# agnusmaximus/DistributedMNIST

Hardware: AMD Instinct MI355X
Metric: images/sec (whole node), MNIST CNN sync-SGD (higher is better)
Workload: dtype bf16; 1 GPU; model=lenet, global_batch=1024, parallelism=dp1, mode=full_sync, mode_requested=full_sync, grad_dtype=fp32

## Files before the change

csrc/bindings.cpp:

```cpp

#include <torch/extension.h>
#include <ATen/hip/HIPContext.h>
#include <hip/hip_runtime.h>

#include "kernels.h"

namespace {

#define CHECK_BF16(t) TORCH_CHECK((t).scalar_type() == at::kBFloat16, #t " must be bf16")
#define CHECK_F32(t) TORCH_CHECK((t).scalar_type() == at::kFloat, #t " must be fp32")
#define CHECK_CONTIG(t) TORCH_CHECK((t).is_contiguous(), #t " must be contiguous")
#define CHECK_CUDA(t) TORCH_CHECK((t).is_cuda(), #t " must be on GPU")

const unsigned short* bf16_ptr(const torch::Tensor& t) {
  return reinterpret_cast<const unsigned short*>(t.data_ptr());
}
unsigned short* bf16_mut(torch::Tensor& t) {
  return reinterpret_cast<unsigned short*>(t.data_ptr());
}

hipStream_t cur_stream() {
  return at::hip::getCurrentHIPStream().stream();
}

int cdiv(int a, int b) { return (a + b - 1) / b; }

int pick_splitk(int mtiles, int ntiles, int ksteps) {
  int tiles = mtiles * ntiles;
  if (tiles >= 256 || ksteps <= 1) return 1;
  int want = std::min(ksteps, std::max(1, 512 / tiles));
  return want;
}

int clamp_splitk(int want, int ksteps) {
  int s = std::max(1, std::min(want, ksteps));
  int per = cdiv(ksteps, s);
  return cdiv(ksteps, per);
}

int dw_tr_level() {
  static int v = [] {
    const char* e = getenv("DMNIST_DW_TR");
    return e ? atoi(e) : 1;
  }();
  return v;
}
bool dw_tr_enabled() { return dw_tr_level() != 0; }

bool conv2_dw_slab_route(int H, int W, int Cin, int Cout) {
  return conv2_dw_slab_supported(H, W, Cin, Cout) && dw_tr_enabled() &&
         conv2_dw_slab_enabled() && !getenv("DMNIST_DW_SPREAD");
}

struct DwPlan { int tr, tbm, bn, splitk; };
DwPlan linear_dw_plan(int K, int N, int B) {
  const int ksteps = cdiv(B, 64);
  if (!(dw_tr_enabled() && K % 8 == 0 && N % 64 == 0)) {
    int bm = cdiv(K, 128) * cdiv(N, 128) >= 128 ? 128 : 64;
    int want = pick_splitk(cdiv(K, bm), cdiv(N, bm), cdiv(B, 32));
    return {0, bm, bm, clamp_splitk(want, ksteps)};
  }
  int bn = (N % 128 == 0) ? 128 : 64;
  DwPlan old{1, 128, bn,
             clamp_splitk(pick_splitk(cdiv(K, 128), cdiv(N, bn), cdiv(B, 32)),
                          ksteps)};
  if (const char* e = getenv("DMNIST_DW_PLAN")) {
    int tbm = 0, fbn = 0, sk = 0;
    if (sscanf(e, "%d,%d,%d", &tbm, &fbn, &sk) == 3 &&
        (tbm == 64 || tbm == 128) && (fbn == 64 || fbn == 128) &&
        N % fbn == 0)
      return {1, tbm, fbn, clamp_splitk(sk, ksteps)};
    return old;
  }
  if (cdiv(K, 64) * cdiv(N, 64) >= 256) {
    if (B < 1536) return {1, 64, 64, 1};
    if (B < 6144) return {1, 64, bn, clamp_splitk(2, ksteps)};
  }
  return old;
}

void launch_linear_dw(GemmParams& p, int K, int N, int B, hipStream_t s) {
  DwPlan pl = linear_dw_plan(K, N, B);
  p.splitk = pl.splitk;
  if (pl.tr) {
    bool sw = pl.splitk == 1 && ((uintptr_t)p.C & 15) == 0 && p.ldc % 4 == 0;
    gemm_dw_tr(p, pl.tbm, pl.bn, sw, s);
  } else {
    (pl.tbm == 128 ? gemm_dw_128 : gemm_dw_64)(p, s);
  }
}

torch::Tensor linear_act_fwd_impl(torch::Tensor x, torch::Tensor w,
                                  torch::Tensor b, bool relu, double p_keep,
                                  int64_t seed, int64_t offset,
                                  const long* offset_dev,
                                  const c10::optional<torch::Tensor>& wT) {
  CHECK_CUDA(x); CHECK_BF16(x); CHECK_CONTIG(x);
  CHECK_BF16(w); CHECK_CONTIG(w);
  CHECK_F32(b); CHECK_CONTIG(b);
  int M = x.size(0), K = x.size(1), N = w.size(1);
  TORCH_CHECK(w.size(0) == K, "w/x shape mismatch");
  auto y = torch::empty({M, N}, x.options());
  GemmParams p{};
  p.A = bf16_ptr(x);
  p.bias = b.data_ptr<float>();
  p.C = y.data_ptr(); p.amax = nullptr;
  p.M = M; p.N = N; p.K = K;
  p.lda = K; p.ldc = N;
  p.splitk = 1;
  p.p_keep = (float)p_keep; p.seed = (uint64_t)seed; p.offset = (uint64_t)offset;
  p.offset_dev = offset_dev;
  bool drop = p_keep < 1.0;
  TORCH_CHECK(!drop || relu, "dropout path requires relu epilogue");
  int g128 = cdiv(M, 128) * cdiv(N, 128);
  bool big = g128 >= 512;
  if (const char* e = getenv("DMNIST_FC_TILE")) big = atoi(e) >= 128;
  auto s = cur_stream();
  bool bt = wT.has_value() && wT->defined();
  int tiles64 = cdiv(M, 64) * cdiv(N, 64);
  int ksteps = cdiv(K, 64);
  if (!big && tiles64 < 256 && ksteps >= 16 &&
      !getenv("DMNIST_FC_NOSPLIT")) {
    int sk = std::min(ksteps, std::max(2, 512 / tiles64));
    auto acc = torch::empty({(int64_t)sk, (int64_t)M, (int64_t)N},
                            x.options().dtype(at::kFloat));
    p.C = acc.data_ptr();
    p.splitk = sk;
    const char* fe = getenv("DMNIST_FC_FIXUP");
    bool fixup = fe && atoi(fe) != 0 && N % 8 == 0;
    if (fixup) {
      static std::vector<torch::Tensor>* ws = new std::vector<torch::Tensor>(64);
      int dev = x.get_device();
      TORCH_CHECK(dev >= 0 && dev < 64, "linear_act_fwd: bad device index");
      if (!(*ws)[dev].defined()) {
        hipStreamCaptureStatus cap = hipStreamCaptureStatusNone;
        hipStreamIsCapturing(s, &cap);
        TORCH_CHECK(cap == hipStreamCaptureStatusNone,
                    "linear_act_fwd: first split-K call on a device allocates "
                    "its ticket workspace and must run outside graph capture");
        (*ws)[dev] = torch::zeros({256}, x.options().dtype(at::kInt));
      }
      p.tickets = reinterpret_cast<unsigned*>((*ws)[dev].data_ptr<int>());
      p.Y = bf16_mut(y);
      p.relu = relu ? 1 : 0;
    }
    if (bt) {
      CHECK_BF16((*wT)); CHECK_CONTIG((*wT));
      TORCH_CHECK(wT->size(0) == N && wT->size(1) == K, "wT shape mismatch");
      p.B = bf16_ptr(*wT); p.ldb = K;
      (fixup ? gemm_fwd_slices_fix_64_bt : gemm_fwd_slices_64_bt)(p, s);
    } else {
      p.B = bf16_ptr(w); p.ldb = N;
      (fixup ? gemm_fwd_slices_fix_64 : gemm_fwd_slices_64)(p, s);
    }
    if (!fixup)
      launch_fwd_epilogue(acc.data_ptr<float>(), b.data_ptr<float>(),
                          bf16_mut(y), M, N, sk, relu ? 1 : 0, (float)p_keep,
                          (uint64_t)seed, (uint64_t)offset, offset_dev, s);
    return y;
  }
  if (bt) {
    CHECK_BF16((*wT)); CHECK_CONTIG((*wT));
    TORCH_CHECK(wT->size(0) == N && wT->size(1) == K, "wT shape mismatch");
    p.B = bf16_ptr(*wT); p.ldb = K;
    if (drop) (big ? gemm_fwd_drop_128_bt : gemm_fwd_drop_64_bt)(p, s);
    else if (relu) (big ? gemm_fwd_relu_128_bt : gemm_fwd_relu_64_bt)(p, s);
    else (big ? gemm_fwd_bias_128_bt : gemm_fwd_bias_64_bt)(p, s);
  } else {
    p.B = bf16_ptr(w); p.ldb = N;
    if (drop) (big ? gemm_fwd_drop_128 : gemm_fwd_drop_64)(p, s);
    else if (relu) (big ? gemm_fwd_relu_128 : gemm_fwd_relu_64)(p, s);
    else (big ? gemm_fwd_bias_128 : gemm_fwd_bias_64)(p, s);
  }
  return y;
}

torch::Tensor linear_act_fwd(torch::Tensor x, torch::Tensor w, torch::Tensor b,
                             bool relu, double p_keep, int64_t seed,
                             int64_t offset,
                             c10::optional<torch::Tensor> wT) {
  return linear_act_fwd_impl(x, w, b, relu, p_keep, seed, offset, nullptr, wT);
}

torch::Tensor linear_act_fwd_dev(torch::Tensor x, torch::Tensor w,
                                 torch::Tensor b, bool relu, double p_keep,
                                 int64_t seed, torch::Tensor offset_dev,
                                 c10::optional<torch::Tensor> wT) {
  TORCH_CHECK(offset_dev.scalar_type() == at::kLong && offset_dev.is_cuda(),
              "offset_dev must be a cuda int64 tensor");
  return linear_act_fwd_impl(x, w, b, relu, p_keep, seed, 0,
                             offset_dev.data_ptr<long>(), wT);
}

std::vector<torch::Tensor> linear_act_bwd_impl(torch::Tensor dy, torch::Tensor x,
                                               torch::Tensor w, torch::Tensor y,
                                               bool relu, double p_keep,
                                               bool need_dx,
                                               torch::Tensor dw, torch::Tensor db) {
  CHECK_CUDA(dy); CHECK_BF16(dy); CHECK_CONTIG(dy);
  CHECK_BF16(x); CHECK_CONTIG(x);
  CHECK_BF16(w); CHECK_CONTIG(w);
  int B = x.size(0), K = x.size(1), N = w.size(1);
  auto s = cur_stream();
  if (!db.defined())
    db = torch::zeros({N}, x.options().dtype(at::kFloat));
  CHECK_F32(db); CHECK_CONTIG(db);
  torch::Tensor dyeff;
  bool mask = relu || p_keep < 1.0;
  if (mask) {
    dyeff = torch::empty_like(dy);
    launch_relu_drop_bwd(bf16_ptr(dy), bf16_ptr(y), bf16_mut(dyeff),
                         db.data_ptr<float>(), B, N,
                         (float)(1.0 / p_keep), 1, s);
  } else {
    dyeff = dy;
    launch_relu_drop_bwd(bf16_ptr(dy), bf16_ptr(y), bf16_mut(dyeff),
                         db.data_ptr<float>(), B, N, 1.0f, 0, s);
  }
  if (!dw.defined())
    dw = torch::zeros({K, N}, x.options().dtype(at::kFloat));
  CHECK_F32(dw); CHECK_CONTIG(dw);
  {
    GemmParams p{};
    p.A = bf16_ptr(x); p.B = bf16_ptr(dyeff);
    p.C = dw.data_ptr();
    p.M = K; p.N = N; p.K = B;
    p.lda = K;
    p.ldb = N; p.ldc = N;
    launch_linear_dw(p, K, N, B, s);
  }
  torch::Tensor dx;
  if (need_dx) {
    dx = torch::empty({B, K}, x.options());
    GemmParams p{};
    p.A = bf16_ptr(dyeff); p.B = bf16_ptr(w);
    p.C = dx.data_ptr();
    p.M = B; p.N = K; p.K = N;
    p.lda = N; p.ldb = N; p.ldc = K;
    p.splitk = 1;
    bool big = cdiv(B, 128) * cdiv(K, 128) >= 128;
    (big ? gemm_dx_128 : gemm_dx_64)(p, s);
  } else {
    dx = torch::empty({0}, x.options());
  }
  return {dx, dw, db};
}

std::vector<torch::Tensor> linear_act_bwd(torch::Tensor dy, torch::Tensor x,
                                          torch::Tensor w, torch::Tensor y,
                                          bool relu, double p_keep,
                                          bool need_dx) {
  return linear_act_bwd_impl(dy, x, w, y, relu, p_keep, need_dx,
                             torch::Tensor(), torch::Tensor());
}

torch::Tensor linear_act_bwd_into(torch::Tensor dy, torch::Tensor x,
                                  torch::Tensor w, torch::Tensor y,
                                  bool relu, double p_keep, bool need_dx,
                                  torch::Tensor dw_out, torch::Tensor db_out) {
  auto r = linear_act_bwd_impl(dy, x, w, y, relu, p_keep, need_dx,
                               dw_out.view({x.size(1), w.size(1)}), db_out);
  return r[0];
}

std::vector<torch::Tensor> conv_pool_fwd(torch::Tensor x, torch::Tensor w,
                                         torch::Tensor b,
                                         c10::optional<torch::Tensor> wT) {
  CHECK_CUDA(x); CHECK_BF16(x); CHECK_CONTIG(x);
  CHECK_BF16(w); CHECK_CONTIG(w);
  CHECK_F32(b); CHECK_CONTIG(b);
  int NB = x.size(0), H = x.size(1), W = x.size(2), Cin = x.size(3);
  TORCH_CHECK(w.dim() == 4 && w.size(0) == 5 && w.size(1) == 5 &&
              w.size(2) == Cin, "conv weight must be [5,5,Cin,Cout]");
  int Cout = w.size(3);
  int Ho = H / 2, Wo = W / 2;
  auto y = torch::empty({NB, Ho, Wo, Cout}, x.options());
  auto amax = torch::empty({NB, Ho, Wo, Cout}, x.options().dtype(at::kByte));
  GemmParams p{};
  p.A = bf16_ptr(x); p.B = bf16_ptr(w);
  p.bias = b.data_ptr<float>();
  p.C = y.data_ptr(); p.amax = amax.data_ptr<uint8_t>();
  p.M = NB * Ho * Wo * 4; p.N = Cout; p.K = 25 * Cin;
  p.ldb = Cout; p.ldc = Cout;
  p.splitk = 1;
  p.CB = NB; p.CH = H; p.CW = W; p.CHo = Ho; p.CWo = Wo;
  p.Cin = Cin; p.Cout = Cout;
  auto s = cur_stream();
  if (Cin == 1 && conv1_mfma_supported(H, W, Cin, Cout) &&
      conv1_mfma_enabled() &&
      reinterpret_cast<uintptr_t>(x.data_ptr()) % 8 == 0) {
    launch_conv1_mfma_fwd(bf16_ptr(x), bf16_ptr(w), b.data_ptr<float>(),
                          bf16_mut(y), amax.data_ptr<uint8_t>(), NB, s);
  } else if (Cin == 1) {
    launch_conv1_direct_fwd(bf16_ptr(x), bf16_ptr(w), b.data_ptr<float>(),
                            bf16_mut(y), amax.data_ptr<uint8_t>(), NB, H, W,
                            Cout, s);
  } else if (conv_slab_supported(H, W, Cin, Cout)) {
    launch_conv_fwd_slab(bf16_ptr(x), bf16_ptr(w), b.data_ptr<float>(),
                         bf16_mut(y), amax.data_ptr<uint8_t>(), NB, H, W,
                         Cin, Cout, s);
  } else {
    TORCH_CHECK(Cin % 8 == 0, "conv requires Cin==1 or Cin%8==0");
    if (wT.has_value() && wT->defined()) {
      CHECK_BF16((*wT)); CHECK_CONTIG((*wT));
      p.B = bf16_ptr(*wT); p.ldb = 25 * Cin;
      conv_fwd_pool_bt(p, s);
    } else {
      conv_fwd_pool(p, s);
    }
  }
  return {y, amax};
}

std::vector<torch::Tensor> conv_pool_bwd_impl(torch::Tensor dy, torch::Tensor x,
                                              torch::Tensor w, torch::Tensor y,
                                              torch::Tensor amax, bool need_dx,
                                              torch::Tensor dw, torch::Tensor db) {
  CHECK_CUDA(dy); CHECK_BF16(dy); CHECK_CONTIG(dy);
  CHECK_BF16(x); CHECK_CONTIG(x); CHECK_BF16(w); CHECK_CONTIG(w);
  int NB = x.size(0), H = x.size(1), W = x.size(2), Cin = x.size(3);
  int Cout = w.size(3);
  int Ho = H / 2, Wo = W / 2;
  auto s = cur_stream();
  auto dact = torch::empty({NB, H, W, Cout}, x.options());
  if (!db.defined())
    db = torch::zeros({Cout}, x.options().dtype(at::kFloat));
  CHECK_F32(db); CHECK_CONTIG(db);
  launch_pool_bwd_scatter(bf16_ptr(dy), bf16_ptr(y),
                          amax.data_ptr<uint8_t>(), bf16_mut(dact),
                          db.data_ptr<float>(), NB * Ho * Wo, Cout, H, W, Wo,
                          s);
  if (!dw.defined())
    dw = torch::zeros({5, 5, Cin, Cout}, x.options().dtype(at::kFloat));
  CHECK_F32(dw); CHECK_CONTIG(dw);
  {
    GemmParams p{};
    p.A = bf16_ptr(x); p.B = bf16_ptr(dact);
    p.C = dw.data_ptr();
    p.M = 25 * Cin; p.N = Cout; p.K = NB * H * W;
    p.ldb = Cout; p.ldc = Cout;
    p.CB = NB; p.CH = H; p.CW = W; p.Cin = Cin; p.Cout = Cout;
    if (Cin == 1 && H <= 28 && W <= 28 && Cout <= 32 &&
        !getenv("DMNIST_DW1_SLAB")) {
      launch_conv1_dw_direct(bf16_ptr(x), bf16_ptr(dact),
                             dw.data_ptr<float>(), NB, H, W, Cout, s);
    } else if (Cin == 1 && conv1_slab_supported(H, W, Cin, Cout)) {
      launch_conv1_dw_slab(bf16_ptr(x), bf16_ptr(dact), dw.data_ptr<float>(),
                           NB, H, W, Cout, s);
    } else if (Cin == 1) {
      p.splitk = std::min(cdiv(p.K, 64), 2048);
      conv1_dw_gemm(p, s);
    } else if (conv_slab_supported(H, W, Cin, Cout) &&
               ((dw_tr_level() == 0 && NB >= 2048) || getenv("DMNIST_DW_G"))) {
      launch_conv_dw_slab(bf16_ptr(x), bf16_ptr(dact), dw.data_ptr<float>(),
                          NB, H, W, Cin, Cout, s);
    } else if (conv2_dw_slab_route(H, W, Cin, Cout)) {
      launch_conv2_dw_slab(bf16_ptr(x), bf16_ptr(dact), dw.data_ptr<float>(),
                           NB, s);
    } else {
      int tiles = cdiv(p.M, 128) * cdiv(p.N, 64);
      int want = p.K <= 262144 ? 1024 : 2048;
      if (const char* e = getenv("DMNIST_DW_BLOCKS")) want = atoi(e);
      p.splitk = std::min(cdiv(p.K, 64), std::max(1, want / tiles));
      if (dw_tr_enabled() && Cin % 8 == 0 && Cout % 64 == 0)
        conv_dw_tr(p, s);
      else
        conv_dw_gemm(p, s);
    }
  }
  torch::Tensor dx;
  if (need_dx && conv_slab_supported(H, W, Cin, Cout)) {
    dx = torch::empty({NB, H, W, Cin}, x.options());
    launch_conv_dx_slab(bf16_ptr(dact), bf16_ptr(w), bf16_mut(dx), NB, H, W,
                        Cin, Cout, s);
  } else if (need_dx) {
    TORCH_CHECK(Cout % 32 == 0, "conv_dx requires Cout%32==0");
    dx = torch::empty({NB, H, W, Cin}, x.options());
    GemmParams p{};
    p.A = bf16_ptr(dact); p.B = bf16_ptr(w);
    p.C = dx.data_ptr();
    p.M = NB * H * W; p.N = Cin; p.K = 25 * Cout;
    p.ldc = Cin;
    p.CB = NB; p.CH = H; p.CW = W; p.Cin = Cin; p.Cout = Cout;
    p.splitk = 1;
    conv_dx_gemm(p, s);
  } else {
    dx = torch::empty({0}, x.options());
  }
  return {dx, dw, db};
}

std::vector<torch::Tensor> conv_pool_bwd(torch::Tensor dy, torch::Tensor x,
                                         torch::Tensor w, torch::Tensor y,
                                         torch::Tensor amax, bool need_dx) {
  return conv_pool_bwd_impl(dy, x, w, y, amax, need_dx, torch::Tensor(),
                            torch::Tensor());
}

torch::Tensor conv_pool_bwd_into(torch::Tensor dy, torch::Tensor x,
                                 torch::Tensor w, torch::Tensor y,
                                 torch::Tensor amax, bool need_dx,
                                 torch::Tensor dw_out, torch::Tensor db_out) {
  auto r = conv_pool_bwd_impl(dy, x, w, y, amax, need_dx,
                              dw_out.view_as(w), db_out);
  return r[0];
}

torch::Tensor mask_db(torch::Tensor dy, torch::Tensor y, bool relu,
                      double p_keep, torch::Tensor db_out) {
  CHECK_CUDA(dy); CHECK_BF16(dy); CHECK_CONTIG(dy);
  CHECK_F32(db_out); CHECK_CONTIG(db_out);
  int B = dy.size(0), N = dy.size(1);
  auto s = cur_stream();
  bool mask = relu || p_keep < 1.0;
  torch::Tensor dyeff = mask ? torch::empty_like(dy) : dy;
  launch_relu_drop_bwd(bf16_ptr(dy), mask ? bf16_ptr(y) : bf16_ptr(dy),
                       bf16_mut(dyeff), db_out.data_ptr<float>(), B, N,
                       (float)(1.0 / p_keep), mask ? 1 : 0, s);
  return dyeff;
}

void linear_dw_into(torch::Tensor x, torch::Tensor dyeff,
                    torch::Tensor dw_out) {
  CHECK_BF16(x); CHECK_CONTIG(x); CHECK_BF16(dyeff); CHECK_CONTIG(dyeff);
  CHECK_F32(dw_out);
  int B = x.size(0), K = x.size(1), N = dyeff.size(1);
  GemmParams p{};
  p.A = bf16_ptr(x); p.B = bf16_ptr(dyeff);
  p.C = dw_out.data_ptr();
  p.M = K; p.N = N; p.K = B;
  p.lda = K; p.ldb = N; p.ldc = N;
  launch_linear_dw(p, K, N, B, cur_stream());
}

torch::Tensor linear_dx(torch::Tensor dyeff, torch::Tensor w) {
  CHECK_BF16(dyeff); CHECK_CONTIG(dyeff); CHECK_BF16(w); CHECK_CONTIG(w);
  int B = dyeff.size(0), N = dyeff.size(1), K = w.size(0);
  auto dx = torch::empty({B, K}, dyeff.options());
  GemmParams p{};
  p.A = bf16_ptr(dyeff); p.B = bf16_ptr(w);
  p.C = dx.data_ptr();
  p.M = B; p.N = K; p.K = N;
  p.lda = N; p.ldb = N; p.ldc = K;
  p.splitk = 1;
  bool big = cdiv(B, 128) * cdiv(K, 128) >= 128;
  (big ? gemm_dx_128 : gemm_dx_64)(p, cur_stream());
  return dx;
}

torch::Tensor linear_dx_unpool(torch::Tensor dyeff, torch::Tensor w,
                               torch::Tensor amax, torch::Tensor db_out,
                               int64_t Ho, int64_t Wo, int64_t C) {
  CHECK_BF16(dyeff); CHECK_CONTIG(dyeff); CHECK_BF16(w); CHECK_CONTIG(w);
  int B = dyeff.size(0), N = dyeff.size(1), K = w.size(0);
  TORCH_CHECK(K == Ho * Wo * C, "linear_dx_unpool: K != Ho*Wo*C");
  auto dact = torch::empty({B, 2 * (int)Ho, 2 * (int)Wo, (int)C},
                           dyeff.options());
  GemmParams p{};
  p.A = bf16_ptr(dyeff); p.B = bf16_ptr(w);
  p.C = dact.data_ptr();
  p.M = B; p.N = K; p.K = N;
  p.lda = N; p.ldb = N; p.ldc = K;
  p.splitk = 1;
  p.CHo = Ho; p.CWo = Wo; p.Cout = C;
  p.amax = amax.data_ptr<uint8_t>();
  p.db = db_out.defined() ? db_out.data_ptr<float>() : nullptr;
  const char* le = getenv("DMNIST_UNPOOL_LINES");
  p.unpool_lines = !(le && atoi(le) == 0) && C % 64 == 0 &&
                   ((uintptr_t)p.amax & 15) == 0 && ((uintptr_t)p.C & 15) == 0;
  bool big = cdiv(B, 128) * cdiv(K, 128) >= (p.unpool_lines ? 400 : 512);
  if (const char* e = getenv("DMNIST_UNPOOL_TILE")) big = atoi(e) >= 128;
  (big ? gemm_dx_unpool_128 : gemm_dx_unpool_64)(p, cur_stream());
  return dact;
}

torch::Tensor linear_dx_mask(torch::Tensor dyeff, torch::Tensor w,
                             torch::Tensor actm, torch::Tensor db_out,
                             double p_keep) {
  CHECK_BF16(dyeff); CHECK_CONTIG(dyeff); CHECK_BF16(w); CHECK_CONTIG(w);
  CHECK_BF16(actm); CHECK_CONTIG(actm);
  int B = dyeff.size(0), N = dyeff.size(1), K = w.size(0);
  TORCH_CHECK(actm.size(0) == B && actm.size(1) == K, "actm shape mismatch");
  auto dx = torch::empty({B, K}, dyeff.options());
  GemmParams p{};
  p.A = bf16_ptr(dyeff); p.B = bf16_ptr(w);
  p.C = dx.data_ptr();
  p.M = B; p.N = K; p.K = N;
  p.lda = N; p.ldb = N; p.ldc = K;
  p.splitk = 1;
  p.p_keep = (float)(1.0 / p_keep);
  p.actm = bf16_ptr(actm);
  p.db = db_out.defined() ? db_out.data_ptr<float>() : nullptr;
  bool big = cdiv(B, 128) * cdiv(K, 128) >= 128;
  (big ? gemm_dx_mask_128 : gemm_dx_mask_64)(p, cur_stream());
  return dx;
}

torch::Tensor pool_scatter(torch::Tensor dy, torch::Tensor y,
                           torch::Tensor amax, torch::Tensor db_out,
                           int64_t H, int64_t W) {
  CHECK_BF16(dy); CHECK_CONTIG(dy);
  int NB = dy.size(0), Ho = dy.size(1), Wo = dy.size(2), C = dy.size(3);
  auto dact = torch::empty({NB, (int)H, (int)W, C}, dy.options());
  launch_pool_bwd_scatter(bf16_ptr(dy), bf16_ptr(y),
                          amax.data_ptr<uint8_t>(), bf16_mut(dact),
                          db_out.data_ptr<float>(), NB * Ho * Wo, C, H, W,
                          Wo, cur_stream());
  return dact;
}

void conv_dw_into(torch::Tensor x, torch::Tensor dact, torch::Tensor dw_out) {
  CHECK_BF16(x); CHECK_CONTIG(x); CHECK_BF16(dact); CHECK_CONTIG(dact);
  int NB = x.size(0), H = x.size(1), W = x.size(2), Cin = x.size(3);
  int Cout = dact.size(3);
  auto s = cur_stream();
  GemmParams p{};
  p.A = bf16_ptr(x); p.B = bf16_ptr(dact);
  p.C = dw_out.data_ptr();
  p.M = 25 * Cin; p.N = Cout; p.K = NB * H * W;
  p.ldb = Cout; p.ldc = Cout;
  p.CB = NB; p.CH = H; p.CW = W; p.Cin = Cin; p.Cout = Cout;
  if (Cin == 1 && H <= 28 && W <= 28 && Cout <= 32 &&
      !getenv("DMNIST_DW1_SLAB")) {
    launch_conv1_dw_direct(bf16_ptr(x), bf16_ptr(dact),
                           dw_out.data_ptr<float>(), NB, H, W, Cout, s);
  } else if (Cin == 1 && conv1_slab_supported(H, W, Cin, Cout)) {
    launch_conv1_dw_slab(bf16_ptr(x), bf16_ptr(dact),
                         dw_out.data_ptr<float>(), NB, H, W, Cout, s);
  } else if (Cin == 1) {
    p.splitk = std::min(cdiv(p.K, 64), 2048);
    conv1_dw_gemm(p, s);
  } else if (conv_slab_supported(H, W, Cin, Cout) &&
             ((dw_tr_level() == 0 && NB >= 2048) || getenv("DMNIST_DW_G"))) {
    launch_conv_dw_slab(bf16_ptr(x), bf16_ptr(dact), dw_out.data_ptr<float>(),
                        NB, H, W, Cin, Cout, s);
  } else if (conv2_dw_slab_route(H, W, Cin, Cout)) {
    launch_conv2_dw_slab(bf16_ptr(x), bf16_ptr(dact),
                         dw_out.data_ptr<float>(), NB, s);
  } else {
    int tiles = cdiv(p.M, 128) * cdiv(p.N, 64);
    int want = p.K <= 262144 ? 1024 : 2048;
    if (const char* e = getenv("DMNIST_DW_BLOCKS")) want = atoi(e);
    p.splitk = std::min(cdiv(p.K, 64), std::max(1, want / tiles));
    if (getenv("DMNIST_DW_SPREAD")) {
      static torch::Tensor scratch;
      int64_t need = 16LL * p.M * p.N;
      if (!scratch.defined() || scratch.numel() < need)
        scratch = torch::zeros({need}, dact.options().dtype(at::kFloat));
      p.C = scratch.data_ptr();
      p.offset = 1;
    }
    if (dw_tr_enabled() && Cin % 8 == 0 && Cout % 64 == 0)
      conv_dw_tr(p, s);
    else
      conv_dw_gemm(p, s);
  }
}

void conv1_dw_pooled(torch::Tensor x, torch::Tensor dyp, torch::Tensor am,
                     torch::Tensor dw_out, torch::Tensor db_out) {
  CHECK_BF16(x); CHECK_CONTIG(x);
  CHECK_BF16(dyp); CHECK_CONTIG(dyp);
  int NB = x.size(0), H = x.size(1), W = x.size(2);
  int Cout = dyp.size(3);
  TORCH_CHECK(x.size(3) == 1 && H == 28 && W == 28 && Cout == 32 &&
                  dyp.size(1) == H / 2 && dyp.size(2) == W / 2,
              "conv1_dw_pooled: LeNet conv1 shapes only");
  CHECK_CONTIG(am); CHECK_F32(dw_out); CHECK_CONTIG(dw_out);
  if (conv1_mfma_supported(H, W, 1, Cout) && conv1_mfma_enabled() &&
      reinterpret_cast<uintptr_t>(x.data_ptr()) % 8 == 0) {
    launch_conv1_mfma_dw(bf16_ptr(x), bf16_ptr(dyp), am.data_ptr<uint8_t>(),
                         dw_out.data_ptr<float>(),
                         db_out.defined() ? db_out.data_ptr<float>() : nullptr,
                         NB, cur_stream());
    return;
  }
  launch_conv1_dw_pooled(bf16_ptr(x), bf16_ptr(dyp),
                         am.data_ptr<uint8_t>(), dw_out.data_ptr<float>(),
                         db_out.defined() ? db_out.data_ptr<float>() : nullptr,
                         NB, H, W, Cout, cur_stream());
}

torch::Tensor conv_dx(torch::Tensor dact, torch::Tensor w, int64_t Cin) {
  CHECK_BF16(dact); CHECK_CONTIG(dact); CHECK_BF16(w); CHECK_CONTIG(w);
  int NB = dact.size(0), H = dact.size(1), W = dact.size(2),
      Cout = dact.size(3);
  auto s = cur_stream();
  auto dx = torch::empty({NB, H, W, (int)Cin}, dact.options());
  if (conv_slab_supported(H, W, Cin, Cout)) {
    launch_conv_dx_slab(bf16_ptr(dact), bf16_ptr(w), bf16_mut(dx), NB, H, W,
                        Cin, Cout, s);
  } else {
    TORCH_CHECK(Cout % 32 == 0, "conv_dx requires Cout%32==0");
    GemmParams p{};
    p.A = bf16_ptr(dact); p.B = bf16_ptr(w);
    p.C = dx.data_ptr();
    p.M = NB * H * W; p.N = Cin; p.K = 25 * Cout;
    p.ldc = Cin;
    p.CB = NB; p.CH = H; p.CW = W; p.Cin = Cin; p.Cout = Cout;
    p.splitk = 1;
    conv_dx_gemm(p, s);
  }
  return dx;
}

std::vector<torch::Tensor> softmax_xent_fwd(torch::Tensor logits,
                                            torch::Tensor labels,
                                            c10::optional<torch::Tensor> db_out,
                                            double inv_n) {
  CHECK_CUDA(logits); CHECK_BF16(logits); CHECK_CONTIG(logits);
  TORCH_CHECK(labels.scalar_type() == at::kLong, "labels must be int64");
  CHECK_CONTIG(labels);
  int B = logits.size(0), C = logits.size(1);
  TORCH_CHECK(C <= 16, "softmax_xent kernel supports C<=16");
  TORCH_CHECK(B <= 256 * SOFTMAX_MAX_BLOCKS, "softmax_xent: batch too large");
  auto dl = torch::empty_like(logits);
  auto out = torch::empty({2}, logits.options().dtype(at::kFloat));
  static std::vector<torch::Tensor>* ws = new std::vector<torch::Tensor>(64);
  int dev = logits.get_device();
  TORCH_CHECK(dev >= 0 && dev < 64, "softmax_xent: bad device index");
  if (!(*ws)[dev].defined()) {
    hipStreamCaptureStatus cap = hipStreamCaptureStatusNone;
    hipStreamIsCapturing(cur_stream(), &cap);
    TORCH_CHECK(cap == hipStreamCaptureStatusNone,
                "softmax_xent_fwd: first call on a device allocates its "
                "workspace and must run outside graph capture");
    (*ws)[dev] = torch::zeros({2 * SOFTMAX_MAX_BLOCKS + 1},
                              logits.options().dtype(at::kFloat));
  }
  float* part = (*ws)[dev].data_ptr<float>();
  unsigned* ticket = reinterpret_cast<unsigned*>(part + 2 * SOFTMAX_MAX_BLOCKS);
  float* dbp = nullptr;
  if (db_out.has_value() && db_out->defined())
    dbp = db_out->data_ptr<float>();
  launch_softmax_xent(bf16_ptr(logits), labels.data_ptr<long>(),
                      bf16_mut(dl), out.data_ptr<float>(), B, C, dbp,
                      (float)inv_n, part, ticket, cur_stream());
  auto loss = out.select(0, 0);
  auto correct = out.select(0, 1);
  return {loss, correct, dl};
}

void sgd_step(torch::Tensor master, torch::Tensor grad, torch::Tensor shadow,
              bool has_shadow, double lr, double scale, double dc_keep,
              int64_t seed, int64_t offset,
              c10::optional<torch::Tensor> momentum, double mu) {
  CHECK_CUDA(master); CHECK_F32(master); CHECK_CONTIG(master);
  CHECK_F32(grad); CHECK_CONTIG(grad);
  float* mom = nullptr;
  if (momentum.has_value() && momentum->defined()) {
    CHECK_F32((*momentum)); CHECK_CONTIG((*momentum));
    mom = momentum->data_ptr<float>();
  }
  launch_sgd_step(master.data_ptr<float>(), grad.data_ptr<float>(),
                  has_shadow ? bf16_mut(shadow) : nullptr,
                  has_shadow ? 1 : 0, master.numel(),
                  (float)(lr * scale), (float)dc_keep, (uint64_t)seed,
                  (uint64_t)offset, mom, (float)mu, cur_stream());
}

void sgd_step_dev(torch::Tensor master, torch::Tensor grad,
                  torch::Tensor shadow, bool has_shadow,
                  torch::Tensor lr_scale_dev, double dc_keep, int64_t seed,
                  torch::Tensor offset_dev,
                  c10::optional<torch::Tensor> momentum, double mu,
                  bool zero_grad) {
  CHECK_CUDA(master); CHECK_F32(master); CHECK_CONTIG(master);
  CHECK_F32(grad); CHECK_CONTIG(grad);
  CHECK_F32(lr_scale_dev);
  float* mom = nullptr;
  if (momentum.has_value() && momentum->defined()) {
    CHECK_F32((*momentum)); CHECK_CONTIG((*momentum));
    mom = momentum->data_ptr<float>();
  }
  launch_sgd_step_dev(master.data_ptr<float>(), grad.data_ptr<float>(),
                      has_shadow ? bf16_mut(shadow) : nullptr,
                      has_shadow ? 1 : 0, master.numel(),
                      lr_scale_dev.data_ptr<float>(), (float)dc_keep,
                      (uint64_t)seed, offset_dev.data_ptr<long>(),
                      mom, (float)mu, zero_grad ? 1 : 0, cur_stream());
}

void transpose_bf16_batch(std::vector<torch::Tensor> srcs,
                          std::vector<torch::Tensor> dsts) {
  TORCH_CHECK(srcs.size() == dsts.size() && srcs.size() <= 4,
              "up to 4 transpose pairs");
  TransposeDesc d[4];
  for (size_t i = 0; i < srcs.size(); ++i) {
    CHECK_BF16(srcs[i]); CHECK_CONTIG(srcs[i]);
    CHECK_BF16(dsts[i]); CHECK_CONTIG(dsts[i]);
    d[i] = {bf16_ptr(srcs[i]), bf16_mut(dsts[i]),
            (int)srcs[i].size(0), (int)srcs[i].size(1)};
  }
  launch_transpose_bf16_batch(d, (int)srcs.size(), cur_stream());
}

void transpose_bf16_batch_adv(std::vector<torch::Tensor> srcs,
                              std::vector<torch::Tensor> dsts,
                              torch::Tensor step_dev,
                              torch::Tensor lr_scale_dev, double lr0,
                              double decay, int64_t decay_steps,
                              double inv_contrib) {
  TORCH_CHECK(srcs.size() == dsts.size() && srcs.size() <= 4,
              "up to 4 transpose pairs");
  TransposeDesc d[4];
  for (size_t i = 0; i < srcs.size(); ++i) {
    CHECK_BF16(srcs[i]); CHECK_CONTIG(srcs[i]);
    CHECK_BF16(dsts[i]); CHECK_CONTIG(dsts[i]);
    d[i] = {bf16_ptr(srcs[i]), bf16_mut(dsts[i]),
            (int)srcs[i].size(0), (int)srcs[i].size(1)};
  }
  launch_transpose_bf16_batch_adv(
      d, (int)srcs.size(), step_dev.data_ptr<long>(),
      lr_scale_dev.data_ptr<float>(), (float)lr0, (float)decay,
      (int)decay_steps, (float)inv_contrib, cur_stream());
}

void transpose_bf16(torch::Tensor src, torch::Tensor dst) {
  CHECK_CUDA(src); CHECK_BF16(src); CHECK_CONTIG(src);
  CHECK_BF16(dst); CHECK_CONTIG(dst);
  TORCH_CHECK(src.dim() == 2 && dst.size(0) == src.size(1) &&
              dst.size(1) == src.size(0), "transpose shape mismatch");
  launch_transpose_bf16(bf16_ptr(src), bf16_mut(dst), src.size(0),
                        src.size(1), cur_stream());
}

void step_advance(torch::Tensor step_dev, torch::Tensor lr_scale_dev,
                  double lr0, double decay, int64_t decay_steps,
                  double inv_contrib) {
  launch_step_advance(step_dev.data_ptr<long>(),
                      lr_scale_dev.data_ptr<float>(), (float)lr0,
                      (float)decay, (int)decay_steps, (float)inv_contrib,
                      cur_stream());
}

void grad_mask(torch::Tensor g, double keep, int64_t seed, int64_t step,
               int64_t rank, int64_t base,
               c10::optional<torch::Tensor> step_dev) {
  CHECK_CUDA(g); CHECK_F32(g); CHECK_CONTIG(g);
  TORCH_CHECK(base % 4 == 0,
              "grad_mask: slice base must be 16B-aligned so slice-wise "
              "masks compose to the whole-buffer mask");
  const long* sd = nullptr;
  if (step_dev.has_value() && step_dev->defined())
    sd = step_dev->data_ptr<long>();
  launch_grad_mask(g.data_ptr<float>(), g.numel(), base, (float)keep,
                   (uint64_t)seed, (uint64_t)step, (uint64_t)rank, sd,
                   cur_stream());
}

void batch_gather(torch::Tensor img_u8, torch::Tensor lab_u8,
                  torch::Tensor lut, torch::Tensor x, torch::Tensor y,
                  int64_t seed, int64_t step,
                  c10::optional<torch::Tensor> step_dev) {
  CHECK_CUDA(img_u8); CHECK_CONTIG(img_u8);
  CHECK_CUDA(lab_u8); CHECK_CONTIG(lab_u8);
  CHECK_CUDA(lut); CHECK_BF16(lut); CHECK_CONTIG(lut);
  CHECK_CUDA(x); CHECK_BF16(x); CHECK_CONTIG(x);
  CHECK_CUDA(y); CHECK_CONTIG(y);
  TORCH_CHECK(img_u8.scalar_type() == at::kByte &&
              lab_u8.scalar_type() == at::kByte,
              "batch_gather: images/labels must be uint8");
  TORCH_CHECK(y.scalar_type() == at::kLong, "batch_gather: y must be int64");
  const int64_t N = lab_u8.numel(), B = y.numel();
  TORCH_CHECK(N >= 1 && N < (int64_t(1) << 31),
              "batch_gather: N out of range");
  TORCH_CHECK(B >= 1 && B <= N, "batch_gather: batch size ", B,
              " must be in [1, N=", N, "]");
  TORCH_CHECK(img_u8.numel() == N * 784, "batch_gather: images must be [N,784]");
  TORCH_CHECK(x.numel() == B * 784, "batch_gather: x must hold B*784 values");
  TORCH_CHECK(lut.numel() == 256, "batch_gather: lut must have 256 entries");
  TORCH_CHECK(reinterpret_cast<uintptr_t>(img_u8.data_ptr()) % 8 == 0 &&
              reinterpret_cast<uintptr_t>(x.data_ptr()) % 16 == 0,
              "batch_gather: images must be 8B- and x 16B-aligned");
  const long* sd = nullptr;
  if (step_dev.has_value() && step_dev->defined()) {
    TORCH_CHECK(step_dev->is_cuda() && step_dev->scalar_type() == at::kLong &&
                step_dev->numel() >= 1, "batch_gather: step_dev must be a "
                "device int64 tensor");
    sd = step_dev->data_ptr<long>();
  } else {
    TORCH_CHECK(step >= 0, "batch_gather: step must be >= 0");
  }
  launch_batch_gather(img_u8.data_ptr<uint8_t>(), lab_u8.data_ptr<uint8_t>(),
                      bf16_ptr(lut), bf16_mut(x), y.data_ptr<long>(),
                      (uint32_t)N, (uint32_t)B, (uint64_t)seed,
                      (uint64_t)step, sd, cur_stream());
}

void batch_gather_aug(torch::Tensor img_u8, torch::Tensor lab_u8,
                      torch::Tensor lut, torch::Tensor table, torch::Tensor x,
                      torch::Tensor y, int64_t seed, int64_t step,
                      c10::optional<torch::Tensor> step_dev) {
  CHECK_CUDA(img_u8); CHECK_CONTIG(img_u8);
  CHECK_CUDA(lab_u8); CHECK_CONTIG(lab_u8);
  CHECK_CUDA(lut); CHECK_BF16(lut); CHECK_CONTIG(lut);
  CHECK_CUDA(table); CHECK_CONTIG(table);
  CHECK_CUDA(x); CHECK_BF16(x); CHECK_CONTIG(x);
  CHECK_CUDA(y); CHECK_CONTIG(y);
  TORCH_CHECK(img_u8.scalar_type() == at::kByte &&
              lab_u8.scalar_type() == at::kByte,
              "batch_gather_aug: images/labels must be uint8");
  TORCH_CHECK(y.scalar_type() == at::kLong,
              "batch_gather_aug: y must be int64");
  TORCH_CHECK(table.scalar_type() == at::kInt && table.dim() == 2 &&
              table.size(1) == 6 && table.size(0) >= 1 &&
              table.size(0) < (int64_t(1) << 31),
              "batch_gather_aug: table must be int32 [T >= 1, 6]");
  const int64_t N = lab_u8.numel(), B = y.numel();
  TORCH_CHECK(N >= 1 && N < (int64_t(1) << 31),
              "batch_gather_aug: N out of range");
  TORCH_CHECK(B >= 1 && B <= N, "batch_gather_aug: batch size ", B,
              " must be in [1, N=", N, "]");
  TORCH_CHECK(img_u8.numel() == N * 784,
              "batch_gather_aug: images must be [N,784]");
  TORCH_CHECK(x.numel() == B * 784,
              "batch_gather_aug: x must hold B*784 values");
  TORCH_CHECK(lut.numel() == 256,
              "batch_gather_aug: lut must have 256 entries");
  TORCH_CHECK(reinterpret_cast<uintptr_t>(img_u8.data_ptr()) % 8 == 0 &&
              reinterpret_cast<uintptr_t>(x.data_ptr()) % 16 == 0,
              "batch_gather_aug: images must be 8B- and x 16B-aligned");
  const long* sd = nullptr;
  if (step_dev.has_value() && step_dev->defined()) {
    TORCH_CHECK(step_dev->is_cuda() && step_dev->scalar_type() == at::kLong &&
                step_dev->numel() >= 1, "batch_gather_aug: step_dev must be "
                "a device int64 tensor");
    sd = step_dev->data_ptr<long>();
  } else {
    TORCH_CHECK(step >= 0, "batch_gather_aug: step must be >= 0");
  }
  launch_batch_gather_aug(img_u8.data_ptr<uint8_t>(),
                          lab_u8.data_ptr<uint8_t>(), bf16_ptr(lut),
                          table.data_ptr<int>(), (uint32_t)table.size(0),
                          bf16_mut(x), y.data_ptr<long>(), (uint32_t)N,
                          (uint32_t)B, (uint64_t)seed, (uint64_t)step, sd,
                          cur_stream());
}

void range_gather(torch::Tensor img_u8, torch::Tensor lab_u8,
                  torch::Tensor lut, torch::Tensor x, torch::Tensor y,
                  int64_t start, c10::optional<torch::Tensor> start_dev) {
  CHECK_CUDA(img_u8); CHECK_CONTIG(img_u8);
  CHECK_CUDA(lab_u8); CHECK_CONTIG(lab_u8);
  CHECK_CUDA(lut); CHECK_BF16(lut); CHECK_CONTIG(lut);
  CHECK_CUDA(x); CHECK_BF16(x); CHECK_CONTIG(x);
  CHECK_CUDA(y); CHECK_CONTIG(y);
  TORCH_CHECK(img_u8.scalar_type() == at::kByte &&
              lab_u8.scalar_type() == at::kByte,
              "range_gather: images/labels must be uint8");
  TORCH_CHECK(y.scalar_type() == at::kLong, "range_gather: y must be int64");
  const int64_t N = lab_u8.numel(), B = y.numel();
  TORCH_CHECK(N >= 1 && N < (int64_t(1) << 31),
              "range_gather: N out of range");
  TORCH_CHECK(B >= 1 && B < (int64_t(1) << 31),
              "range_gather: chunk size out of range");
  TORCH_CHECK(img_u8.numel() == N * 784, "range_gather: images must be [N,784]");
  TORCH_CHECK(x.numel() == B * 784, "range_gather: x must hold B*784 values");
  TORCH_CHECK(lut.numel() == 256, "range_gather: lut must have 256 entries");
  TORCH_CHECK(reinterpret_cast<uintptr_t>(img_u8.data_ptr()) % 8 == 0 &&
              reinterpret_cast<uintptr_t>(x.data_ptr()) % 16 == 0,
              "range_gather: images must be 8B- and x 16B-aligned");
  const long* sd = nullptr;
  if (start_dev.has_value() && start_dev->defined()) {
    TORCH_CHECK(start_dev->is_cuda() && start_dev->scalar_type() == at::kLong &&
                start_dev->numel() >= 1, "range_gather: start_dev must be a "
                "device int64 tensor");
    sd = start_dev->data_ptr<long>();
  } else {
    TORCH_CHECK(start >= 0, "range_gather: start must be >= 0");
  }
  launch_range_gather(img_u8.data_ptr<uint8_t>(), lab_u8.data_ptr<uint8_t>(),
                      bf16_ptr(lut), bf16_mut(x), y.data_ptr<long>(),
                      (uint32_t)N, (uint32_t)B, (uint64_t)start, sd,
                      cur_stream());
}

void softmax_eval(torch::Tensor logits, torch::Tensor labels,
                  torch::Tensor loss_sum, torch::Tensor counts,
                  c10::optional<torch::Tensor> pred,
                  c10::optional<torch::Tensor> cursor_dev) {
  CHECK_CUDA(logits); CHECK_BF16(logits); CHECK_CONTIG(logits);
  CHECK_CUDA(labels); CHECK_CONTIG(labels);
  CHECK_CUDA(loss_sum); CHECK_F32(loss_sum); CHECK_CONTIG(loss_sum);
  CHECK_CUDA(counts); CHECK_CONTIG(counts);
  TORCH_CHECK(logits.dim() == 2, "softmax_eval: logits must be [B,C]");
  TORCH_CHECK(labels.scalar_type() == at::kLong,
              "softmax_eval: labels must be int64");
  TORCH_CHECK(counts.scalar_type() == at::kInt,
              "softmax_eval: counts must be int32");
  const int64_t B = logits.size(0), C = logits.size(1);
  TORCH_CHECK(C >= 1 && C <= 16, "softmax_eval kernel supports 1<=C<=16");
  TORCH_CHECK(B >= 1 && B <= 256 * SOFTMAX_MAX_BLOCKS,
              "softmax_eval: batch out of range");
  TORCH_CHECK(labels.numel() == B, "softmax_eval: labels must be [B]");
  TORCH_CHECK(loss_sum.numel() >= 1, "softmax_eval: loss_sum must be [1]");
  TORCH_CHECK(counts.numel() == 2 + C * C,
              "softmax_eval: counts must hold 2 + C*C = ", 2 + C * C,
              " values");
  uint8_t* pp = nullptr;
  if (pred.has_value() && pred->defined()) {
    TORCH_CHECK(pred->is_cuda() && pred->scalar_type() == at::kByte &&
                pred->is_contiguous() && pred->numel() == B,
                "softmax_eval: pred must be a contiguous device uint8 [B]");
    pp = pred->data_ptr<uint8_t>();
  }
  long* cp = nullptr;
  if (cursor_dev.has_value() && cursor_dev->defined()) {
    TORCH_CHECK(cursor_dev->is_cuda() &&
                cursor_dev->scalar_type() == at::kLong &&
                cursor_dev->numel() >= 1, "softmax_eval: cursor_dev must be "
                "a device int64 tensor");
    cp = cursor_dev->data_ptr<long>();
  }
  static std::vector<torch::Tensor>* ws = new std::vector<torch::Tensor>(64);
  int dev = logits.get_device();
  TORCH_CHECK(dev >= 0 && dev < 64, "softmax_eval: bad device index");
  if (!(*ws)[dev].defined()) {
    hipStreamCaptureStatus cap = hipStreamCaptureStatusNone;
    hipStreamIsCapturing(cur_stream(), &cap);
    TORCH_CHECK(cap == hipStreamCaptureStatusNone,
                "softmax_eval: first call on a device allocates its "
                "workspace and must run outside graph capture");
    (*ws)[dev] = torch::zeros({SOFTMAX_MAX_BLOCKS + 1},
                              logits.options().dtype(at::kFloat));
  }
  float* part = (*ws)[dev].data_ptr<float>();
  unsigned* ticket = reinterpret_cast<unsigned*>(part + SOFTMAX_MAX_BLOCKS);
  launch_softmax_eval(bf16_ptr(logits), labels.data_ptr<long>(),
                      loss_sum.data_ptr<float>(), counts.data_ptr<int>(), pp,
                      cp, (int)B, (int)C, part, ticket, cur_stream());
}

}

PYBIND11_MODULE(TORCH_EXTENSION_NAME, m) {
  m.def("linear_act_fwd", &linear_act_fwd, "fused linear+bias+relu+dropout",
        py::arg("x"), py::arg("w"), py::arg("b"), py::arg("relu"),
        py::arg("p_keep"), py::arg("seed"), py::arg("offset"),
        py::arg("wT") = c10::nullopt);
  m.def("transpose_bf16", &transpose_bf16, "bf16 2-D transpose (wT refresh)");
  m.def("transpose_bf16_batch_adv", &transpose_bf16_batch_adv,
        "batched transposes + fused device step/LR advance (graph tail)");
  m.def("transpose_bf16_batch", &transpose_bf16_batch,
        "up to 4 transposes in one launch");
  m.def("mask_db", &mask_db, "relu/dropout grad mask + bias-grad column sums");
  m.def("linear_dw_into", &linear_dw_into, "dW = x^T dyeff into bucket view");
  m.def("linear_dx", &linear_dx, "dx = dyeff @ W^T");
  m.def("linear_dx_mask", &linear_dx_mask,
        "dx GEMM with fused relu/dropout mask + bias-grad column sums",
        py::arg("dyeff"), py::arg("w"), py::arg("actm"), py::arg("db_out"),
        py::arg("p_keep"));
  m.def("linear_dx_unpool", &linear_dx_unpool,
        "dx GEMM fused with maxpool2x2 backward scatter + conv db",
        py::arg("dyeff"), py::arg("w"), py::arg("amax"),
        py::arg("db_out"), py::arg("Ho"), py::arg("Wo"), py::arg("C"));
  m.def("linear_dw_plan", [](int64_t K, int64_t N, int64_t B) {
    DwPlan pl = linear_dw_plan((int)K, (int)N, (int)B);
    return std::make_tuple(pl.tbm, pl.bn, pl.splitk);
  }, "(tbm, bn, splitk) the fc dW launcher picks for x[B,K], dyeff[B,N]");
  m.def("pool_scatter", &pool_scatter, "maxpool bwd scatter + conv db");
  m.def("conv_dw_into", &conv_dw_into, "conv dW into bucket view");
  m.def("conv1_dw_pooled", &conv1_dw_pooled,
        "conv1 dW+db from the pooled gradient (pool bwd fused, no dact1)",
        py::arg("x"), py::arg("dyp"), py::arg("am"),
        py::arg("dw_out"), py::arg("db_out"));
  m.def("conv1_dw_group", [](int64_t NB) {
          return (int64_t)conv1_mfma_dw_group((int)NB);
        }, "images per block the MFMA conv1 dW launcher picks for batch NB");
  m.def("conv2_dw_group", [](int64_t NB) {
          return (int64_t)conv2_dw_group((int)NB);
        }, "images per block the slab conv2 dW launcher picks for batch NB");
  m.def("conv_dx", &conv_dx, "conv dX");
  m.def("linear_act_bwd", &linear_act_bwd, "linear backward (dx, dw, db)");
  m.def("linear_act_bwd_into", &linear_act_bwd_into,
        "linear backward accumulating dw/db into bucket views");
  m.def("conv_pool_fwd", &conv_pool_fwd, "fused conv5x5+bias+relu+maxpool",
        py::arg("x"), py::arg("w"), py::arg("b"), py::arg("wT") = c10::nullopt);
  m.def("conv_pool_bwd", &conv_pool_bwd, "conv+pool backward (dx, dw, db)");
  m.def("conv_pool_bwd_into", &conv_pool_bwd_into,
        "conv backward accumulating dw/db into bucket views");
  m.def("softmax_xent_fwd", &softmax_xent_fwd, "fused softmax-CE (+grad, +optional fc2 db, +optional acc-mean scale)",
        py::arg("logits"), py::arg("labels"),
        py::arg("db_out") = c10::nullopt, py::arg("inv_n") = 1.0);
  m.def("sgd_step", &sgd_step, "fused flat SGD(+momentum) apply",
        py::arg("master"), py::arg("grad"), py::arg("shadow"),
        py::arg("has_shadow"), py::arg("lr"), py::arg("scale"),
        py::arg("dc_keep"), py::arg("seed"), py::arg("offset"),
        py::arg("momentum") = c10::nullopt, py::arg("mu") = 0.0);
  m.def("sgd_step_dev", &sgd_step_dev,
        "SGD apply with device-side lr/offset (hipGraph-capturable); "
        "zero_grad clears the bucket in the same pass",
        py::arg("master"), py::arg("grad"), py::arg("shadow"),
        py::arg("has_shadow"), py::arg("lr_scale_dev"), py::arg("dc_keep"),
        py::arg("seed"), py::arg("offset_dev"),
        py::arg("momentum") = c10::nullopt, py::arg("mu") = 0.0,
        py::arg("zero_grad") = false);
  m.def("step_advance", &step_advance,
        "device-side staircase LR + step increment (inside the graph)");
  m.def("grad_mask", &grad_mask,
        "per-rank pre-aggregation drop-connect mask (in-place, philox; "
        "reference distributed_train.py:194-203)",
        py::arg("g"), py::arg("keep"), py::arg("seed"), py::arg("step"),
        py::arg("rank"), py::arg("base") = 0,
        py::arg("step_dev") = c10::nullopt);
  m.def("batch_gather", &batch_gather,
        "gather one training batch from the device-resident uint8 set "
        "(Feistel epoch permutation keyed on seed + step; LUT-normalised "
        "to bf16) into x [B,28,28,1] bf16 / y [B] int64",
        py::arg("img_u8"), py::arg("lab_u8"), py::arg("lut"), py::arg("x"),
        py::arg("y"), py::arg("seed"), py::arg("step"),
        py::arg("step_dev") = c10::nullopt);
  m.def("batch_gather_aug", &batch_gather_aug,
        "batch_gather with on-device affine augmentation: image j is warped "
        "(integer bilinear, zero background) by row aug_indices(seed, step, "
        "j) of the int32 [T,6] Q16 inverse-affine table before the LUT",
        py::arg("img_u8"), py::arg("lab_u8"), py::arg("lut"),
        py::arg("table"), py::arg("x"), py::arg("y"), py::arg("seed"),
        py::arg("step"), py::arg("step_dev") = c10::nullopt);
  m.def("range_gather", &range_gather,
        "sequential chunk [start, start+B) of the device-resident uint8 set "
        "(LUT-normalised to bf16) into x [B,28,28,1] bf16 / y [B] int64; "
        "rows past N are zero-filled with label -1",
        py::arg("img_u8"), py::arg("lab_u8"), py::arg("lut"), py::arg("x"),
        py::arg("y"), py::arg("start"),
        py::arg("start_dev") = c10::nullopt);
  m.def("softmax_eval", &softmax_eval,
        "evaluation statistics accumulated across launches: loss_sum[1] "
        "fp32, counts[2 + C*C] int32 (live, correct, confusion), optional "
        "pred[B] uint8 and cursor_dev += B; rows with a label outside "
        "[0, C) contribute to nothing",
        py::arg("logits"), py::arg("labels"), py::arg("loss_sum"),
        py::arg("counts"), py::arg("pred") = c10::nullopt,
        py::arg("cursor_dev") = c10::nullopt);
  m.def("linear_act_fwd_dev", &linear_act_fwd_dev,
        "linear fwd with device-side dropout offset",
        py::arg("x"), py::arg("w"), py::arg("b"), py::arg("relu"),
        py::arg("p_keep"), py::arg("seed"), py::arg("offset_dev"),
        py::arg("wT") = c10::nullopt);
}
```

csrc/common.h:

```cpp
#pragma once

#include <hip/hip_runtime.h>
#include <hip/hip_bf16.h>
#include <stdint.h>

typedef __attribute__((ext_vector_type(8))) short short8;
typedef __attribute__((ext_vector_type(4))) float f32x4;
typedef unsigned short ushort_t;

#define DEV __device__ __forceinline__

DEV float bf2f(ushort_t u) {
  union { uint32_t i; float f; } v;
  v.i = uint32_t(u) << 16;
  return v.f;
}

DEV ushort_t f2bf(float f) {
  union { float f; uint32_t i; } v;
  v.f = f;
  uint32_t lsb = (v.i >> 16) & 1;
  uint32_t rounded = v.i + 0x7FFFu + lsb;
  if ((v.i & 0x7F800000u) == 0x7F800000u) rounded = v.i;
  return ushort_t(rounded >> 16);
}

struct Philox4 {
  uint32_t x, y, z, w;
};

DEV uint32_t mulhilo(uint32_t a, uint32_t b, uint32_t* hi) {
  uint64_t p = uint64_t(a) * uint64_t(b);
  *hi = uint32_t(p >> 32);
  return uint32_t(p);
}

DEV Philox4 philox4x32(uint64_t seed, uint64_t offset, uint64_t idx) {
  uint32_t k0 = uint32_t(seed), k1 = uint32_t(seed >> 32);
  uint32_t c0 = uint32_t(idx), c1 = uint32_t(idx >> 32);
  uint32_t c2 = uint32_t(offset), c3 = uint32_t(offset >> 32);
  const uint32_t M0 = 0xD2511F53u, M1 = 0xCD9E8D57u;
  const uint32_t W0 = 0x9E3779B9u, W1 = 0xBB67AE85u;
#pragma unroll
  for (int r = 0; r < 10; ++r) {
    uint32_t h0, h1;
    uint32_t l0 = mulhilo(M0, c0, &h0);
    uint32_t l1 = mulhilo(M1, c2, &h1);
    uint32_t n0 = h1 ^ c1 ^ k0;
    uint32_t n1 = l1;
    uint32_t n2 = h0 ^ c3 ^ k1;
    uint32_t n3 = l0;
    c0 = n0; c1 = n1; c2 = n2; c3 = n3;
    k0 += W0; k1 += W1;
  }
  return {c0, c1, c2, c3};
}

DEV float philox_uniform(uint64_t seed, uint64_t offset, uint64_t idx) {
  Philox4 p = philox4x32(seed, offset, idx);
  return float(p.x) * (1.0f / 4294967296.0f);
}

DEV int cdiv(int a, int b) { return (a + b - 1) / b; }

DEV void glds16(const ushort_t* src, ushort_t* dst) {
  __builtin_amdgcn_global_load_lds(src, dst, 16, 0, 0);
}

DEV uint2 tr16_issue(unsigned a) {
  uint2 d;
  asm volatile("ds_read_b64_tr_b16 %0, %1 offset:0"
               : "=&v"(d) : "v"(a) : "memory");
  return d;
}

DEV short8 pack_wait(uint2 lo, uint2 hi) {
  union { unsigned u[4]; short8 s; } r;
  r.u[0] = lo.x; r.u[1] = lo.y; r.u[2] = hi.x; r.u[3] = hi.y;
  asm volatile("s_waitcnt lgkmcnt(0)" : "+v"(r.s));
  return r.s;
}

typedef short bf16x2_t __attribute__((__vector_size__(2 * sizeof(short))));
DEV float dot2bf(unsigned a, unsigned b, float c) {
  union U { unsigned u; bf16x2_t v; };
  U ua, ub;
  ua.u = a; ub.u = b;
  return __builtin_amdgcn_fdot2_f32_bf16(ua.v, ub.v, c, false);
}
```

csrc/conv2_dw_slab.hip:

```cpp

#include "common.h"
#include "kernels.h"
#include <stdlib.h>
#include <stdexcept>

#define C2_MG 8
#define C2_XIMG (14 * 14 * 32)
#define C2_DIMG (14 * 14 * 64)

static __device__ __align__(16) unsigned short c2_zero_page[8];

DEV int c2_xswz(int s) { return ((s >> 3) & 1) << 1; }
DEV int c2_dswz(int k) { return (((k >> 1) & 1) | (((k >> 3) & 1) << 1)) << 1; }

extern __shared__ __align__(16) ushort_t c2_lds[];

template <int KHB, int NBUF>
__global__ __launch_bounds__(256, (KHB == 1 && NBUF == 1) ? 3 : 1)
void conv2_dw_slab_kernel(const ushort_t* __restrict__ x,
                          const ushort_t* __restrict__ dact,
                          float* __restrict__ dw, int NB, int G) {
  constexpr int NRX = 13 + KHB;
  constexpr int XPIX = C2_MG + NRX * 16 + C2_MG;
  constexpr int NJOB = NRX + 28;
  constexpr int NQ = (NJOB + 3) / 4;
  constexpr int NKB = 5 / KHB;
  constexpr int KS_UNROLL = KHB == 1 ? 7 : 1;
  constexpr int BUF = XPIX * 32 + 224 * 64;
  ushort_t* const X = c2_lds;
  ushort_t* const D = c2_lds + XPIX * 32;

  const int tid = threadIdx.x;
  const int lane = tid & 63, wave = tid >> 6;
  const int wr = wave >> 1, wc = wave & 1;

  const int pos = blockIdx.x >> 3;
  const int grp = (pos / NKB) * 8 + (blockIdx.x & 7);
  const int kh0 = (pos % NKB) * KHB;
  const int img0 = grp * G;
  if (img0 >= NB) return;

  if (tid < 64 * NBUF) {
    int t = tid & 63;
    int o = (t < 32) ? t * 8 : (C2_MG + NRX * 16) * 32 + (t - 32) * 8;
    *reinterpret_cast<short8*>(X + (tid >> 6) * BUF + o) =
        short8{0, 0, 0, 0, 0, 0, 0, 0};
  }

  int soff[NQ];
#pragma unroll
  for (int q = 0; q < NQ; ++q) {
    int j = wave + 4 * q;
    soff[q] = -1;
    if (j < NRX) {
      int ir = j + kh0 - 2, px = lane >> 2;
      int lc = (lane & 3) ^ c2_xswz(C2_MG + j * 16 + px);
      if (px < 14 && ir >= 0 && ir < 14) soff[q] = (ir * 14 + px) * 32 + lc * 8;
    } else if (j < NJOB) {
      int jj = j - NRX;
      int h = jj >> 1, px = (jj & 1) * 8 + (lane >> 3);
      int lc = (lane & 7) ^ c2_dswz(h * 16 + px);
      if (px < 14) soff[q] = (h * 14 + px) * 64 + lc * 8;
    }
  }
  const auto issue = [&](int buf, int img) {
    const ushort_t* xi = x + (size_t)img * C2_XIMG;
    const ushort_t* di = dact + (size_t)img * C2_DIMG;
#pragma unroll
    for (int q = 0; q < NQ; ++q) {
      int j = wave + 4 * q;
      if (j < NRX) {
        const ushort_t* src = soff[q] >= 0 ? xi + soff[q] : c2_zero_page;
        glds16(src, X + buf * BUF + (C2_MG + j * 16) * 32);
      } else if (j < NJOB) {
        const ushort_t* src = soff[q] >= 0 ? di + soff[q] : c2_zero_page;
        glds16(src, D + buf * BUF + (j - NRX) * 8 * 64);
      }
    }
  };

  const int r0 = (lane >> 4) * 8 + ((lane & 15) >> 2);
  const int cp = (lane & 3) >> 1, off8 = (lane & 1) * 8;
  unsigned aaddr[5][2], baddr[2][2];
#pragma unroll
  for (int kw = 0; kw < 5; ++kw)
#pragma unroll
    for (int t = 0; t < 2; ++t) {
      int s = C2_MG + r0 + 4 * t + kw - 2;
      aaddr[kw][t] = (unsigned)(uintptr_t)X +
                     (unsigned)(s * 64 + (((wr * 2 + cp) ^ c2_xswz(s)) << 4) +
                                off8);
    }
#pragma unroll
  for (int ni = 0; ni < 2; ++ni)
#pragma unroll
    for (int t = 0; t < 2; ++t) {
      int k = r0 + 4 * t;
      baddr[ni][t] = (unsigned)(uintptr_t)D +
                     (unsigned)(k * 128 +
                                (((wc * 4 + ni * 2 + cp) ^ c2_dswz(k)) << 4) +
                                off8);
    }

  f32x4 acc[KHB][5][2];
#pragma unroll
  for (int a = 0; a < KHB; ++a)
#pragma unroll
    for (int b = 0; b < 5; ++b)
#pragma unroll
      for (int c = 0; c < 2; ++c) acc[a][b][c] = f32x4{0.f, 0.f, 0.f, 0.f};

  const int n = min(G, NB - img0);
  if (NBUF == 2) issue(0, img0);
  for (int g = 0; g < n; ++g) {
    if (NBUF == 1) {
      __syncthreads();
      issue(0, img0 + g);
    }
    asm volatile("s_waitcnt vmcnt(0)" ::: "memory");
    __syncthreads();
    if (NBUF == 2 && g + 1 < n) issue((g + 1) & 1, img0 + g + 1);
    const unsigned boff = (unsigned)((g & (NBUF - 1)) * BUF * 2);
#pragma unroll KS_UNROLL
    for (int ks = 0; ks < 7; ++ks) {
      uint2 br[2][2];
#pragma unroll
      for (int ni = 0; ni < 2; ++ni)
#pragma unroll
        for (int t = 0; t < 2; ++t)
          br[ni][t] = tr16_issue(baddr[ni][t] + boff + ks * (32 * 128));
#pragma unroll
      for (int khl = 0; khl < KHB; ++khl) {
        uint2 ar[5][2];
#pragma unroll
        for (int kw = 0; kw < 5; ++kw)
#pragma unroll
          for (int t = 0; t < 2; ++t)
            ar[kw][t] = tr16_issue(aaddr[kw][t] + boff +
                                   (ks * 32 + khl * 16) * 64);
        short8 af[5], bf[2];
#pragma unroll
        for (int kw = 0; kw < 5; ++kw) af[kw] = pack_wait(ar[kw][0], ar[kw][1]);
#pragma unroll
        for (int ni = 0; ni < 2; ++ni) bf[ni] = pack_wait(br[ni][0], br[ni][1]);
#pragma unroll
        for (int kw = 0; kw < 5; ++kw)
#pragma unroll
          for (int ni = 0; ni < 2; ++ni)
            acc[khl][kw][ni] = __builtin_amdgcn_mfma_f32_16x16x32_bf16(
                af[kw], bf[ni], acc[khl][kw][ni], 0, 0, 0);
      }
    }
  }

  const int frow = (lane >> 4) * 4, fcol = lane & 15;
#pragma unroll
  for (int khl = 0; khl < KHB; ++khl)
#pragma unroll
    for (int kw = 0; kw < 5; ++kw)
#pragma unroll
      for (int ni = 0; ni < 2; ++ni)
#pragma unroll
        for (int r = 0; r < 4; ++r) {
          int m = ((kh0 + khl) * 5 + kw) * 32 + wr * 16 + frow + r;
          int n = wc * 32 + ni * 16 + fcol;
          atomicAdd(dw + m * 64 + n, acc[khl][kw][ni][r]);
        }
}


bool conv2_dw_slab_supported(int H, int W, int Cin, int Cout) {
  return H == 14 && W == 14 && Cin == 32 && Cout == 64;
}

bool conv2_dw_slab_enabled() {
  const char* e = getenv("DMNIST_DW2_SLAB");
  return !(e && atoi(e) == 0);
}

int conv2_dw_group(int NB) {
  int G = NB >= 4096 ? 32 : (NB >= 512 ? 12 : (NB >= 128 ? 4 : 1));
  if (const char* e = getenv("DMNIST_DW2_G")) G = atoi(e);
  return G < 1 ? 1 : G;
}

template <int KHB, int NBUF>
static void c2_launch(const unsigned short* x, const unsigned short* dact,
                      float* dw, int NB, int G, int blocks, hipStream_t s) {
  constexpr int BYTES = NBUF * ((C2_MG * 2 + (13 + KHB) * 16) * 32 + 224 * 64) * 2;
  if (BYTES > 65536) {
    static const hipError_t granted = hipFuncSetAttribute(
        reinterpret_cast<const void*>(&conv2_dw_slab_kernel<KHB, NBUF>),
        hipFuncAttributeMaxDynamicSharedMemorySize, BYTES);
    if (granted != hipSuccess)
      throw std::runtime_error("conv2_dw_slab: LDS size not granted");
  }
  hipLaunchKernelGGL((conv2_dw_slab_kernel<KHB, NBUF>), dim3(blocks),
                     dim3(256), BYTES, s, x, dact, dw, NB, G);
}

void launch_conv2_dw_slab(const unsigned short* x, const unsigned short* dact,
                          float* dw, int NB, hipStream_t s) {
  if (NB <= 0) return;
  int G = conv2_dw_group(NB);
  int groups = (NB + G - 1) / G;
  int g8 = (groups + 7) / 8 * 8;
  const char* e = getenv("DMNIST_DW2_KHB");
  const char* b = getenv("DMNIST_DW2_NBUF");
  bool all_taps = e && atoi(e) == 5;
  int nbuf = b ? atoi(b) : 1;
  if (all_taps && nbuf == 2)
    c2_launch<5, 2>(x, dact, dw, NB, G, g8, s);
  else if (all_taps)
    c2_launch<5, 1>(x, dact, dw, NB, G, g8, s);
  else if (nbuf == 2)
    c2_launch<1, 2>(x, dact, dw, NB, G, g8 * 5, s);
  else
    c2_launch<1, 1>(x, dact, dw, NB, G, g8 * 5, s);
}
```

csrc/conv_slab.hip:

```cpp

#include "common.h"
#include "kernels.h"
#include <stdlib.h>

#define NTHREADS 256
#define BK 64
#define LDK (BK + 8)

typedef ushort_t u16;

__device__ __align__(16) static unsigned short g_zero_page_slab[8];

DEV short8 lds_row_shifted(const u16* row, int s) {
  int s0 = s & ~7;
  short8 lo = *reinterpret_cast<const short8*>(row + s0);
  short8 hi = *reinterpret_cast<const short8*>(row + s0 + 8);
  switch (s & 7) {
    case 0: return lo;
    case 1: return __builtin_shufflevector(lo, hi, 1, 2, 3, 4, 5, 6, 7, 8);
    case 2: return __builtin_shufflevector(lo, hi, 2, 3, 4, 5, 6, 7, 8, 9);
    case 3: return __builtin_shufflevector(lo, hi, 3, 4, 5, 6, 7, 8, 9, 10);
    case 4: return __builtin_shufflevector(lo, hi, 4, 5, 6, 7, 8, 9, 10, 11);
    case 5: return __builtin_shufflevector(lo, hi, 5, 6, 7, 8, 9, 10, 11, 12);
    case 6: return __builtin_shufflevector(lo, hi, 6, 7, 8, 9, 10, 11, 12, 13);
    default: return __builtin_shufflevector(lo, hi, 7, 8, 9, 10, 11, 12, 13, 14);
  }
}

template <int H, int W, int CIN, int COUT>
__global__ __launch_bounds__(NTHREADS)
void conv_fwd_slab_kernel(const u16* __restrict__ x,
                          const u16* __restrict__ w,
                          const float* __restrict__ bias, u16* __restrict__ y,
                          uint8_t* __restrict__ amax, int NB) {
  constexpr int HP = H + 4, WP = W + 4;
  constexpr int HO = H / 2, WO = W / 2;
  constexpr int M = HO * WO * 4;
  constexpr int BM = 224;
  constexpr int BN = COUT;
  constexpr int WM = 112, WN = BN / 2;
  constexpr int MI = WM / 16, NI = WN / 16;
  constexpr int K = 25 * CIN;
  constexpr int PST = CIN + 8;
  __shared__ __align__(16) u16 slab[HP * WP * PST];
  __shared__ __align__(16) u16 Bs[2][BK][BN];

  const int tid = threadIdx.x;
  const int lane = tid & 63;
  const int wave = tid >> 6;
  const int wr = wave >> 1, wc = wave & 1;
  const int img = blockIdx.x;
  const u16* xi = x + (size_t)img * H * W * CIN;

  constexpr int BLPR = BN / 8;
  constexpr int BQ = BN / 32;
  int bnc[BQ];
#pragma unroll
  for (int q = 0; q < BQ; ++q) {
    int rt = (wave * BQ + q) * (512 / BN) + lane / BLPR;
    int xs = (rt ^ (rt >> 3)) & (BLPR - 1);
    bnc[q] = ((lane % BLPR) ^ xs) * 8;
  }
  const auto issueB = [&](int buf, int kt) {
#pragma unroll
    for (int q = 0; q < BQ; ++q) {
      int row0 = (wave * BQ + q) * (512 / BN);
      int k = kt + row0 + lane / BLPR;
      const u16* src =
          (k < K) ? w + (size_t)k * COUT + bnc[q] : g_zero_page_slab;
      glds16(src, &Bs[buf][row0][0]);
    }
  };

  for (int c = tid; c < HP * WP * (CIN / 8); c += NTHREADS) {
    int ci = (c % (CIN / 8)) * 8;
    int pix = c / (CIN / 8);
    int xx = pix % WP, yy = pix / WP;
    short8 v = short8{0, 0, 0, 0, 0, 0, 0, 0};
    int sy = yy - 2, sx = xx - 2;
    if (sy >= 0 && sy < H && sx >= 0 && sx < W)
      v = *reinterpret_cast<const short8*>(xi + ((size_t)sy * W + sx) * CIN + ci);
    *reinterpret_cast<short8*>(&slab[(yy * WP + xx) * PST + ci]) = v;
  }

  int arow_off[MI];
#pragma unroll
  for (int mi = 0; mi < MI; ++mi) {
    int lm = wr * WM + mi * 16 + (lane & 15);
    int q = lm >> 2, pos = lm & 3;
    int wo = q % WO, ho = (q / WO) % HO;
    if (lm >= M) { wo = 0; ho = 0; pos = 0; }
    int oy = ho * 2 + (pos >> 1) + 2;
    int ox = wo * 2 + (pos & 1) + 2;
    arow_off[mi] = (oy * WP + ox) * PST;
  }

  f32x4 acc[MI][NI];
#pragma unroll
  for (int mi = 0; mi < MI; ++mi)
#pragma unroll
    for (int ni = 0; ni < NI; ++ni) acc[mi][ni] = f32x4{0.f, 0.f, 0.f, 0.f};

  const int kq = (lane >> 4) * 8;
  const int slot_r = (lane & 15) >> 2;
  const int slot_c = (lane & 3) * 4;
  const int kgrp = (lane >> 4) * 8;
  issueB(0, 0);
  __syncthreads();

  constexpr int NT_K = (K + BK - 1) / BK;
  int cur = 0;
  for (int t = 0; t < NT_K; ++t) {
    int kt = t * BK;
    if (t + 1 < NT_K) issueB(cur ^ 1, kt + BK);
    unsigned bbase = (unsigned)(uintptr_t)&Bs[cur][0][0];
#pragma unroll
    for (int kh2 = 0; kh2 < 2; ++kh2) {
      int kbase = kt + kh2 * 32 + kq;
      int khkw = kbase / CIN, ci = kbase % CIN;
      if (khkw >= 25) { khkw = 0; ci = 0; }
      int kh = khkw / 5, kw = khkw % 5;
      int shift = ((kh - 2) * WP + (kw - 2)) * PST + ci;
      short8 af[MI], bf[NI];
#pragma unroll
      for (int mi = 0; mi < MI; ++mi)
        af[mi] = *reinterpret_cast<const short8*>(
            &slab[arow_off[mi] + shift]);
      uint2 br[NI][2];
#pragma unroll
      for (int ni = 0; ni < NI; ++ni) {
        int cb = (wc * WN + ni * 16 + slot_c) * 2;
        int r0 = kh2 * 32 + kgrp + slot_r;
        int xs0 = (r0 ^ (r0 >> 3)) & (BLPR - 1);
        int r1 = r0 + 4;
        int xs1 = (r1 ^ (r1 >> 3)) & (BLPR - 1);
        br[ni][0] = tr16_issue(bbase + (unsigned)(r0 * (BN * 2) +
                       (((cb >> 4) ^ xs0) << 4) + (cb & 15)));
        br[ni][1] = tr16_issue(bbase + (unsigned)(r1 * (BN * 2) +
                       (((cb >> 4) ^ xs1) << 4) + (cb & 15)));
      }
#pragma unroll
      for (int ni = 0; ni < NI; ++ni) bf[ni] = pack_wait(br[ni][0], br[ni][1]);
#pragma unroll
      for (int mi = 0; mi < MI; ++mi)
#pragma unroll
        for (int ni = 0; ni < NI; ++ni)
          acc[mi][ni] = __builtin_amdgcn_mfma_f32_16x16x32_bf16(
              af[mi], bf[ni], acc[mi][ni], 0, 0, 0);
    }
    __syncthreads();
    cur ^= 1;
  }

  const int frow = (lane >> 4) * 4;
  const int fcol = lane & 15;
  u16* yi = y + (size_t)img * (M / 4) * COUT;
  uint8_t* ai = amax + (size_t)img * (M / 4) * COUT;
#pragma unroll
  for (int mi = 0; mi < MI; ++mi) {
    int lm = wr * WM + mi * 16 + frow;
    if (lm >= M) continue;
    int gq = lm >> 2;
#pragma unroll
    for (int ni = 0; ni < NI; ++ni) {
      int gc = wc * WN + ni * 16 + fcol;
      float bias_v = bias[gc];
      float best = -1.0f / 0.0f;
      int barg = 0;
#pragma unroll
      for (int r = 0; r < 4; ++r) {
        float v = acc[mi][ni][r] + bias_v;
        v = v > 0.f ? v : 0.f;
        if (v > best) { best = v; barg = r; }
      }
      yi[(size_t)gq * COUT + gc] = f2bf(best);
      ai[(size_t)gq * COUT + gc] = (uint8_t)(best > 0.f ? barg : 7);
    }
  }
}

template <int H, int W, int CIN, int COUT, int DB = 2, int PAD = 8>
__global__ __launch_bounds__(NTHREADS)
void conv_dx_slab_kernel(const u16* __restrict__ dact,
                         const u16* __restrict__ w,
                         u16* __restrict__ dx, int NB) {
  constexpr int HP = H + 4, WP = W + 4;
  constexpr int M = H * W;
  constexpr int BM = 224;
  constexpr int BN = CIN;
  constexpr int WM = 112, WN = BN / 2;
  constexpr int MI = WM / 16, NI = WN / 16;
  constexpr int K = 25 * COUT;
  constexpr int PST = COUT + PAD;
  __shared__ __align__(16) u16 slab[HP * WP * PST];
  constexpr int NBUF = (DB >= 2) ? 2 : 1;
  __shared__ __align__(16) u16 Bs[NBUF][BN][BK];

  const int tid = threadIdx.x;
  const int lane = tid & 63;
  const int wave = tid >> 6;
  const int wr = wave >> 1, wc = wave & 1;
  const int img = blockIdx.x;
  const u16* di = dact + (size_t)img * H * W * COUT;

  const int brow = wave * 8 + lane / 8;
  const int bxs = (brow ^ (brow >> 3)) & 7;
  const int blc = (lane % 8) ^ bxs;
  const auto issueB = [&](int buf, int kt) {
    int k = kt + blc * 8;
    const u16* src = g_zero_page_slab;
    if (k < K) {
      int khkw = k / COUT, co = k % COUT;
      src = w + ((size_t)khkw * CIN + brow) * COUT + co;
    }
    glds16(src, &Bs[buf][wave * 8][0]);
  };

  for (int c = tid; c < HP * WP * (COUT / 8); c += NTHREADS) {
    int co = (c % (COUT / 8)) * 8;
    int pix = c / (COUT / 8);
    int xx = pix % WP, yy = pix / WP;
    short8 v = short8{0, 0, 0, 0, 0, 0, 0, 0};
    int sy = yy - 2, sx = xx - 2;
    if (sy >= 0 && sy < H && sx >= 0 && sx < W)
      v = *reinterpret_cast<const short8*>(di + ((size_t)sy * W + sx) * COUT + co);
    *reinterpret_cast<short8*>(&slab[(yy * WP + xx) * PST + co]) = v;
  }

  int arow_off[MI];
#pragma unroll
  for (int mi = 0; mi < MI; ++mi) {
    int lm = wr * WM + mi * 16 + (lane & 15);
    int wi = lm % W, hi = (lm / W) % H;
    if (lm >= M) { wi = 0; hi = 0; }
    arow_off[mi] = ((hi + 2) * WP + (wi + 2)) * PST;
  }

  f32x4 acc[MI][NI];
#pragma unroll
  for (int mi = 0; mi < MI; ++mi)
#pragma unroll
    for (int ni = 0; ni < NI; ++ni) acc[mi][ni] = f32x4{0.f, 0.f, 0.f, 0.f};

  const int kq = (lane >> 4) * 8;
  if (DB == 2) issueB(0, 0);
  __syncthreads();

  constexpr int NT_K = (K + BK - 1) / BK;
  int cur = 0;
  if (DB == 3) {
    for (int t = 0; t < NT_K; t += 2) {
      issueB(0, t * BK);
      if (t + 1 < NT_K) issueB(1, (t + 1) * BK);
      asm volatile("s_waitcnt vmcnt(0)" ::: "memory");
      __syncthreads();
#pragma unroll
      for (int half = 0; half < 2; ++half) {
        if (t + half >= NT_K) break;
        int kt = (t + half) * BK;
        const u16* bp = &Bs[half][0][0];
#pragma unroll
        for (int kh2 = 0; kh2 < 2; ++kh2) {
          int kbase = kt + kh2 * 32 + kq;
          int khkw = kbase / COUT, co = kbase % COUT;
          int kh = khkw / 5, kw = khkw % 5;
          int shift = (-(kh - 2) * WP - (kw - 2)) * PST + co;
          short8 af[MI], bf[NI];
#pragma unroll
          for (int mi = 0; mi < MI; ++mi)
            af[mi] = *reinterpret_cast<const short8*>(
                &slab[arow_off[mi] + shift]);
#pragma unroll
          for (int ni = 0; ni < NI; ++ni) {
            int n = wc * WN + ni * 16 + (lane & 15);
            int xs = (n ^ (n >> 3)) & 7;
            int chunk = (kh2 * 4 + (lane >> 4)) ^ xs;
            bf[ni] = *reinterpret_cast<const short8*>(bp + (size_t)n * BK +
                                                      chunk * 8);
          }
#pragma unroll
          for (int mi = 0; mi < MI; ++mi)
#pragma unroll
            for (int ni = 0; ni < NI; ++ni)
              acc[mi][ni] = __builtin_amdgcn_mfma_f32_16x16x32_bf16(
                  af[mi], bf[ni], acc[mi][ni], 0, 0, 0);
        }
      }
      __syncthreads();
    }
    goto epilogue_dx;
  }
  for (int t = 0; t < NT_K; ++t) {
    int kt = t * BK;
    if (DB == 2) {
      if (t + 1 < NT_K) issueB(cur ^ 1, kt + BK);
    } else {
      issueB(0, kt);
      asm volatile("s_waitcnt vmcnt(0)" ::: "memory");
      __syncthreads();
    }
    const u16* bp = &Bs[cur][0][0];
#pragma unroll
    for (int kh2 = 0; kh2 < 2; ++kh2) {
      int kbase = kt + kh2 * 32 + kq;
      int khkw = kbase / COUT, co = kbase % COUT;
      int kh = khkw / 5, kw = khkw % 5;
      int shift = (-(kh - 2) * WP - (kw - 2)) * PST + co;
      short8 af[MI], bf[NI];
#pragma unroll
      for (int mi = 0; mi < MI; ++mi)
        af[mi] = *reinterpret_cast<const short8*>(
            &slab[arow_off[mi] + shift]);
#pragma unroll
      for (int ni = 0; ni < NI; ++ni) {
        int n = wc * WN + ni * 16 + (lane & 15);
        int xs = (n ^ (n >> 3)) & 7;
        int chunk = (kh2 * 4 + (lane >> 4)) ^ xs;
        bf[ni] = *reinterpret_cast<const short8*>(bp + (size_t)n * BK +
                                                  chunk * 8);
      }
#pragma unroll
      for (int mi = 0; mi < MI; ++mi)
#pragma unroll
        for (int ni = 0; ni < NI; ++ni)
          acc[mi][ni] = __builtin_amdgcn_mfma_f32_16x16x32_bf16(
              af[mi], bf[ni], acc[mi][ni], 0, 0, 0);
    }
    __syncthreads();
    if (DB == 2) cur ^= 1;
  }

epilogue_dx:
  const int frow = (lane >> 4) * 4;
  const int fcol = lane & 15;
  u16* xo = dx + (size_t)img * M * CIN;
#pragma unroll
  for (int mi = 0; mi < MI; ++mi) {
#pragma unroll
    for (int r = 0; r < 4; ++r) {
      int lm = wr * WM + mi * 16 + frow + r;
      if (lm >= M) continue;
#pragma unroll
      for (int ni = 0; ni < NI; ++ni) {
        int gc = wc * WN + ni * 16 + fcol;
        xo[(size_t)lm * CIN + gc] = f2bf(acc[mi][ni][r]);
      }
    }
  }
}

template <int H, int W, int CIN, int COUT>
__global__ __launch_bounds__(NTHREADS)
void conv_dx_slab_hi_occ_kernel(const u16* __restrict__ dact,
                         const u16* __restrict__ w,
                         u16* __restrict__ dx, int NB) {
  constexpr int HP = H + 4, WP = W + 4;
  constexpr int M = H * W;
  constexpr int BM = 224;
  constexpr int BN = CIN;
  constexpr int WM = 112, WN = BN / 2;
  constexpr int MI = WM / 16, NI = WN / 16;
  constexpr int K = 25 * COUT;
  constexpr int PST = COUT + 8;
  __shared__ __align__(16) u16 slab[HP * WP * PST];
  __shared__ __align__(16) u16 Bs[BN][LDK];

  const int tid = threadIdx.x;
  const int lane = tid & 63;
  const int wave = tid >> 6;
  const int wr = wave >> 1, wc = wave & 1;
  const int img = blockIdx.x;
  const u16* di = dact + (size_t)img * H * W * COUT;

  for (int c = tid; c < HP * WP * (COUT / 8); c += NTHREADS) {
    int co = (c % (COUT / 8)) * 8;
    int pix = c / (COUT / 8);
    int xx = pix % WP, yy = pix / WP;
    short8 v = short8{0, 0, 0, 0, 0, 0, 0, 0};
    int sy = yy - 2, sx = xx - 2;
    if (sy >= 0 && sy < H && sx >= 0 && sx < W)
      v = *reinterpret_cast<const short8*>(di + ((size_t)sy * W + sx) * COUT + co);
    *reinterpret_cast<short8*>(&slab[(yy * WP + xx) * PST + co]) = v;
  }

  int arow_off[MI];
#pragma unroll
  for (int mi = 0; mi < MI; ++mi) {
    int lm = wr * WM + mi * 16 + (lane & 15);
    int wi = lm % W, hi = (lm / W) % H;
    if (lm >= M) { wi = 0; hi = 0; }
    arow_off[mi] = ((hi + 2) * WP + (wi + 2)) * PST;
  }

  f32x4 acc[MI][NI];
#pragma unroll
  for (int mi = 0; mi < MI; ++mi)
#pragma unroll
    for (int ni = 0; ni < NI; ++ni) acc[mi][ni] = f32x4{0.f, 0.f, 0.f, 0.f};

  const int kq = (lane >> 4) * 8;
  __syncthreads();

  for (int kt = 0; kt < K; kt += BK) {
    for (int c = tid; c < BN * (BK / 8); c += NTHREADS) {
      int i = c / (BK / 8);
      int kc = (c % (BK / 8)) * 8;
      int k = kt + kc;
      int khkw = k / COUT, co = k % COUT;
      short8 v = *reinterpret_cast<const short8*>(
          w + ((size_t)khkw * CIN + i) * COUT + co);
      *reinterpret_cast<short8*>(&Bs[i][kc]) = v;
    }
    __syncthreads();
#pragma unroll
    for (int kh2 = 0; kh2 < 2; ++kh2) {
      int kbase = kt + kh2 * 32 + kq;
      int khkw = kbase / COUT, co = kbase % COUT;
      int kh = khkw / 5, kw = khkw % 5;
      int shift = (-(kh - 2) * WP - (kw - 2)) * PST + co;
      short8 af[MI], bf[NI];
#pragma unroll
      for (int mi = 0; mi < MI; ++mi)
        af[mi] = *reinterpret_cast<const short8*>(
            &slab[arow_off[mi] + shift]);
#pragma unroll
      for (int ni = 0; ni < NI; ++ni)
        bf[ni] = *reinterpret_cast<const short8*>(
            &Bs[wc * WN + ni * 16 + (lane & 15)][kh2 * 32 + kq]);
#pragma unroll
      for (int mi = 0; mi < MI; ++mi)
#pragma unroll
        for (int ni = 0; ni < NI; ++ni)
          acc[mi][ni] = __builtin_amdgcn_mfma_f32_16x16x32_bf16(
              af[mi], bf[ni], acc[mi][ni], 0, 0, 0);
    }
    __syncthreads();
  }

  const int frow = (lane >> 4) * 4;
  const int fcol = lane & 15;
  u16* xo = dx + (size_t)img * M * CIN;
#pragma unroll
  for (int mi = 0; mi < MI; ++mi) {
#pragma unroll
    for (int r = 0; r < 4; ++r) {
      int lm = wr * WM + mi * 16 + frow + r;
      if (lm >= M) continue;
#pragma unroll
      for (int ni = 0; ni < NI; ++ni) {
        int gc = wc * WN + ni * 16 + fcol;
        xo[(size_t)lm * CIN + gc] = f2bf(acc[mi][ni][r]);
      }
    }
  }
}

void launch_conv_fwd_slab(const unsigned short* x, const unsigned short* w,
                          const float* bias, unsigned short* y, uint8_t* amax,
                          int NB, int H, int W, int Cin, int Cout,
                          hipStream_t s) {
  if (H == 14 && W == 14 && Cin == 32 && Cout == 64) {
    hipLaunchKernelGGL((conv_fwd_slab_kernel<14, 14, 32, 64>), dim3(NB),
                       dim3(NTHREADS), 0, s, x, w, bias, y, amax, NB);
  } else {
  }
}

bool conv_slab_supported(int H, int W, int Cin, int Cout) {
  return H == 14 && W == 14 && Cin == 32 && Cout == 64;
}



void launch_conv_dx_slab(const unsigned short* dact, const unsigned short* w,
                         unsigned short* dx, int NB, int H, int W, int Cin,
                         int Cout, hipStream_t s) {
  if (H == 14 && W == 14 && Cin == 32 && Cout == 64) {
    if (getenv("DMNIST_DX_PAIR"))
      hipLaunchKernelGGL((conv_dx_slab_kernel<14, 14, 32, 64, 3>), dim3(NB),
                         dim3(NTHREADS), 0, s, dact, w, dx, NB);
    else if (NB < 2048)
      hipLaunchKernelGGL((conv_dx_slab_kernel<14, 14, 32, 64, 2>), dim3(NB),
                         dim3(NTHREADS), 0, s, dact, w, dx, NB);
    else if (getenv("DMNIST_DX_HIOCC"))
      hipLaunchKernelGGL((conv_dx_slab_hi_occ_kernel<14, 14, 32, 64>),
                         dim3(NB), dim3(NTHREADS), 0, s, dact, w, dx, NB);
    else if (getenv("DMNIST_DX_DB2SLIM"))
      hipLaunchKernelGGL((conv_dx_slab_kernel<14, 14, 32, 64, 2, 4>),
                         dim3(NB), dim3(NTHREADS), 0, s, dact, w, dx, NB);
    else
      hipLaunchKernelGGL((conv_dx_slab_kernel<14, 14, 32, 64, 1>), dim3(NB),
                         dim3(NTHREADS), 0, s, dact, w, dx, NB);
  }
}

template <int H, int W, int CIN, int COUT, int G, int ABL = 0>
__global__ __launch_bounds__(NTHREADS, 2)
void conv_dw_slab_kernel(const u16* __restrict__ x,
                         const u16* __restrict__ dact,
                         float* __restrict__ dw, int NB) {
  constexpr int HP = H + 4, WP = W + 4;
  constexpr int KPAD = 384;
  constexpr int DST = KPAD + 8;
  constexpr int XROW = 472;
  constexpr int NP = 25 * CIN;
  constexpr int BN = 448;
  constexpr int WN = 112, NI = WN / 16;
  constexpr int MI = COUT / 16;
  __shared__ __align__(16) u16 dslab[COUT][DST];
  __shared__ __align__(16) u16 xslab[CIN][XROW];

  const int tid = threadIdx.x;
  const int lane = tid & 63;
  const int wc = tid >> 6;
  const int img0 = blockIdx.x * G;

  const int lcol = lane & 15;
  const int kq = (lane >> 4) * 8;

  for (int nt = 0; nt < 2; ++nt) {
    f32x4 acc[MI][NI];
#pragma unroll
    for (int mi = 0; mi < MI; ++mi)
#pragma unroll
      for (int ni = 0; ni < NI; ++ni) acc[mi][ni] = f32x4{0.f, 0.f, 0.f, 0.f};

    int bshift[NI];
    int bci[NI];
    bool bvalid[NI];
#pragma unroll
    for (int ni = 0; ni < NI; ++ni) {
      int np = nt * BN + wc * WN + ni * 16 + lcol;
      int khkw = np / CIN, ci = np % CIN;
      bvalid[ni] = np < NP;
      if (!bvalid[ni]) { khkw = 0; ci = 0; }
      bci[ni] = ci;
      bshift[ni] = (khkw / 5) * WP + (khkw % 5);
    }

    __syncthreads();
    for (int c = tid; c < COUT * (DST / 8); c += NTHREADS) {
      *reinterpret_cast<short8*>(&dslab[c / (DST / 8)][(c % (DST / 8)) * 8]) =
          short8{0, 0, 0, 0, 0, 0, 0, 0};
    }
    for (int c = tid; c < CIN * (XROW / 8); c += NTHREADS) {
      *reinterpret_cast<short8*>(&xslab[c / (XROW / 8)][(c % (XROW / 8)) * 8]) =
          short8{0, 0, 0, 0, 0, 0, 0, 0};
    }
    for (int g = 0; g < G; ++g) {
      int img = img0 + g;
      if (img >= NB) break;
      __syncthreads();
      const u16* di = dact + (size_t)img * H * W * COUT;
      const u16* xi = x + (size_t)img * H * W * CIN;
      if (ABL == 2) goto compute;
      for (int c = tid; c < H * W * (COUT / 8); c += NTHREADS) {
        int co0 = (c % (COUT / 8)) * 8;
        int pix = c / (COUT / 8);
        int w_ = pix % W, h_ = pix / W;
        short8 v = *reinterpret_cast<const short8*>(di + (size_t)pix * COUT + co0);
        int pk = (h_ + 2) * WP + (w_ + 2);
#pragma unroll
        for (int e = 0; e < 8; ++e) dslab[co0 + e][pk] = v[e];
      }
      for (int c = tid; c < H * W * (CIN / 8); c += NTHREADS) {
        int ci0 = (c % (CIN / 8)) * 8;
        int pix = c / (CIN / 8);
        int w_ = pix % W, h_ = pix / W;
        short8 v = *reinterpret_cast<const short8*>(xi + (size_t)pix * CIN + ci0);
        int pk = (h_ + 4) * WP + (w_ + 4);
#pragma unroll
        for (int e = 0; e < 8; ++e) xslab[ci0 + e][pk] = v[e];
      }
compute:
      __syncthreads();
      if (ABL == 1) continue;
      for (int kt = 0; kt < KPAD; kt += BK) {
#pragma unroll
        for (int kh2 = 0; kh2 < 2; ++kh2) {
          int k0 = kt + kh2 * 32 + kq;
          short8 af[MI];
#pragma unroll
          for (int mi = 0; mi < MI; ++mi)
            af[mi] = *reinterpret_cast<const short8*>(
                &dslab[mi * 16 + lcol][k0]);
#pragma unroll
          for (int ni = 0; ni < NI; ++ni) {
            short8 bf = lds_row_shifted(&xslab[bci[ni]][0],
                                        bshift[ni] + k0);
#pragma unroll
            for (int mi = 0; mi < MI; ++mi)
              acc[mi][ni] = __builtin_amdgcn_mfma_f32_16x16x32_bf16(
                  af[mi], bf, acc[mi][ni], 0, 0, 0);
          }
        }
      }
    }
    if (ABL == 3) { __syncthreads(); continue; }
#pragma unroll
    for (int mi = 0; mi < MI; ++mi) {
#pragma unroll
      for (int ni = 0; ni < NI; ++ni) {
#pragma unroll
        for (int r = 0; r < 4; ++r) {
          int co = mi * 16 + (lane >> 4) * 4 + r;
          int np = nt * BN + wc * WN + ni * 16 + lcol;
          if (np >= NP) continue;
          int khkw = np / CIN, ci = np % CIN;
          float v = acc[mi][ni][r];
          if (v != 0.f)
            atomicAdd(dw + ((size_t)khkw * CIN + ci) * COUT + co, v);
        }
      }
    }
    __syncthreads();
  }
}

void launch_conv_dw_slab(const unsigned short* x, const unsigned short* dact,
                         float* dw, int NB, int H, int W, int Cin, int Cout,
                         hipStream_t s) {
  if (H == 14 && W == 14 && Cin == 32 && Cout == 64) {
    static int force_g = [] {
      const char* e = getenv("DMNIST_DW_G");
      return e ? atoi(e) : 0;
    }();
    int nb_eff = force_g ? (force_g >= 16 ? 8192 : (force_g >= 4 ? 2048 : 0))
                         : NB;
    static int abl = [] {
      const char* e = getenv("DMNIST_DW_ABL");
      return e ? atoi(e) : 0;
    }();
    if (nb_eff >= 8192) {
      dim3 grid((NB + 15) / 16);
      switch (abl) {
        case 1: hipLaunchKernelGGL((conv_dw_slab_kernel<14, 14, 32, 64, 16, 1>), grid, dim3(NTHREADS), 0, s, x, dact, dw, NB); break;
        case 2: hipLaunchKernelGGL((conv_dw_slab_kernel<14, 14, 32, 64, 16, 2>), grid, dim3(NTHREADS), 0, s, x, dact, dw, NB); break;
        case 3: hipLaunchKernelGGL((conv_dw_slab_kernel<14, 14, 32, 64, 16, 3>), grid, dim3(NTHREADS), 0, s, x, dact, dw, NB); break;
        default: hipLaunchKernelGGL((conv_dw_slab_kernel<14, 14, 32, 64, 16, 0>), grid, dim3(NTHREADS), 0, s, x, dact, dw, NB); break;
      }
    } else if (nb_eff >= 2048) {
      hipLaunchKernelGGL((conv_dw_slab_kernel<14, 14, 32, 64, 4>),
                         dim3((NB + 3) / 4), dim3(NTHREADS), 0, s, x, dact,
                         dw, NB);
    } else {
      hipLaunchKernelGGL((conv_dw_slab_kernel<14, 14, 32, 64, 1>),
                         dim3(NB), dim3(NTHREADS), 0, s, x, dact, dw, NB);
    }
  }
}

template <int H, int W, int COUT, int G>
__global__ __launch_bounds__(NTHREADS, 2)
void conv1_dw_slab_kernel(const u16* __restrict__ x,
                          const u16* __restrict__ dact,
                          float* __restrict__ dw, int NB) {
  constexpr int HP = H + 4, WP = W + 4;
  constexpr int KPAD = HP * WP;
  constexpr int DST = KPAD + 8;
  constexpr int XROW = 1168;
  __shared__ __align__(16) u16 dslab[COUT][DST];
  __shared__ __align__(16) u16 xslab[XROW];

  const int tid = threadIdx.x;
  const int lane = tid & 63;
  const int wave = tid >> 6;
  const int wr = wave >> 1, wc = wave & 1;
  const int img0 = blockIdx.x * G;
  const int lcol = lane & 15;
  const int kq = (lane >> 4) * 8;

  const int khkw = wc * 16 + lcol;
  const int kh = khkw / 5, kw = khkw % 5;
  const int bshift = (khkw < 25) ? kh * WP + kw : 0;

  f32x4 acc = f32x4{0.f, 0.f, 0.f, 0.f};

  for (int c = tid; c < COUT * (DST / 8); c += NTHREADS)
    *reinterpret_cast<short8*>(&dslab[c / (DST / 8)][(c % (DST / 8)) * 8]) =
        short8{0, 0, 0, 0, 0, 0, 0, 0};
  for (int c = tid; c < XROW / 8; c += NTHREADS)
    *reinterpret_cast<short8*>(&xslab[c * 8]) = short8{0, 0, 0, 0, 0, 0, 0, 0};
  for (int g = 0; g < G; ++g) {
    int img = img0 + g;
    if (img >= NB) break;
    __syncthreads();
    const u16* di = dact + (size_t)img * H * W * COUT;
    const u16* xi = x + (size_t)img * H * W;
    for (int c = tid; c < H * W * (COUT / 8); c += NTHREADS) {
      int co0 = (c % (COUT / 8)) * 8;
      int pix = c / (COUT / 8);
      int w_ = pix % W, h_ = pix / W;
      short8 v = *reinterpret_cast<const short8*>(di + (size_t)pix * COUT + co0);
      int pk = (h_ + 2) * WP + (w_ + 2);
#pragma unroll
      for (int e = 0; e < 8; ++e) dslab[co0 + e][pk] = v[e];
    }
    for (int c = tid; c < H * W; c += NTHREADS) {
      int w_ = c % W, h_ = c / W;
      xslab[(h_ + 4) * WP + (w_ + 4)] = xi[c];
    }
    __syncthreads();
    for (int kt = 0; kt < KPAD; kt += BK) {
#pragma unroll
      for (int kh2 = 0; kh2 < 2; ++kh2) {
        int k0 = kt + kh2 * 32 + kq;
        short8 af = *reinterpret_cast<const short8*>(
            &dslab[wr * 16 + lcol][k0]);
        const u16* base = &xslab[bshift + k0];
        short8 bf;
#pragma unroll
        for (int e = 0; e < 8; ++e) bf[e] = (short)base[e];
        acc = __builtin_amdgcn_mfma_f32_16x16x32_bf16(af, bf, acc, 0, 0, 0);
      }
    }
  }
#pragma unroll
  for (int r = 0; r < 4; ++r) {
    int co = wr * 16 + (lane >> 4) * 4 + r;
    if (khkw < 25) {
      float v = acc[r];
      if (v != 0.f) atomicAdd(dw + (size_t)khkw * COUT + co, v);
    }
  }
}

void launch_conv1_dw_slab(const unsigned short* x, const unsigned short* dact,
                          float* dw, int NB, int H, int W, int Cout,
                          hipStream_t s) {
  if (H == 28 && W == 28 && Cout == 32) {
    if (NB >= 4096) {
      hipLaunchKernelGGL((conv1_dw_slab_kernel<28, 28, 32, 8>),
                         dim3((NB + 7) / 8), dim3(NTHREADS), 0, s, x, dact,
                         dw, NB);
    } else {
      hipLaunchKernelGGL((conv1_dw_slab_kernel<28, 28, 32, 2>),
                         dim3((NB + 1) / 2), dim3(NTHREADS), 0, s, x, dact,
                         dw, NB);
    }
  }
}

bool conv1_slab_supported(int H, int W, int Cin, int Cout) {
  return H == 28 && W == 28 && Cin == 1 && Cout == 32;
}
```

csrc/gemm_tile.hip:

```cpp

#include "common.h"
#include "kernels.h"

enum AMode {
  A_N = 0,
  A_T = 1,
  A_CONV_FWD = 2,
  A_CONV1_FWD = 3,
  A_CONV_DX = 4,
  A_CONV_DW = 5,
};
enum BMode {
  B_KMAJ = 0,
  B_NMAJ = 1,
  B_CONV_DX_W = 2,
};
enum Epi { EPI_NONE = 0, EPI_BIAS = 1, EPI_BIAS_RELU = 2, EPI_BIAS_RELU_DROP = 3,
           EPI_POOL = 4, EPI_UNPOOL = 5, EPI_MASK_DB = 6 };
enum OutKind { OUT_BF16 = 0, OUT_F32_ATOMIC = 1, OUT_F32_SLICES = 2,
               OUT_F32_SLICES_FIX = 3 };

#define NTHREADS 256
#define BK 64
#define LDK (BK + 8)

DEV short8 loadRow8(const ushort_t* p, int vcnt) {
  short8 v;
  if (vcnt >= 8 && ((uintptr_t)p & 15) == 0) {
    v = *reinterpret_cast<const short8*>(p);
  } else {
#pragma unroll
    for (int j = 0; j < 8; ++j) v[j] = (j < vcnt) ? (short)p[j] : (short)0;
  }
  return v;
}

DEV bool decode_pool_m(const GemmParams& p, int m, int& n, int& oy, int& ox) {
  int q = m >> 2, pos = m & 3;
  int wo = q % p.CWo;
  int t = q / p.CWo;
  int ho = t % p.CHo;
  n = t / p.CHo;
  oy = ho * 2 + (pos >> 1);
  ox = wo * 2 + (pos & 1);
  return n < p.CB;
}


template <int BM, int AMODE, int CH>
DEV void loadA(const GemmParams& p, int m0, int kt, int kend, int tid,
               short8 (&regs)[CH]) {
#pragma unroll
  for (int j = 0; j < CH; ++j) {
    int c = tid + j * NTHREADS;
    short8 v = short8{0, 0, 0, 0, 0, 0, 0, 0};
    if (AMODE == A_N || AMODE == A_CONV_FWD || AMODE == A_CONV_DX) {
      int i = c / (BK / 8);
      int kc = (c % (BK / 8)) * 8;
      int m = m0 + i, k = kt + kc;
      int vcnt = min(8, kend - k);
      if (m < p.M && vcnt > 0) {
        if (AMODE == A_N) {
          v = loadRow8(p.A + (size_t)m * p.lda + k, vcnt);
        } else if (AMODE == A_CONV_FWD) {
          int khkw = k / p.Cin, ci = k % p.Cin;
          int kh = khkw / 5, kw = khkw % 5;
          int n, oy, ox;
          if (decode_pool_m(p, m, n, oy, ox)) {
            int y = oy + kh - 2, x = ox + kw - 2;
            if (y >= 0 && y < p.CH && x >= 0 && x < p.CW)
              v = loadRow8(p.A + (((size_t)n * p.CH + y) * p.CW + x) * p.Cin + ci,
                           min(vcnt, p.Cin - ci));
          }
        } else {
          int wi = m % p.CW, t2 = m / p.CW;
          int hi = t2 % p.CH, n = t2 / p.CH;
          int khkw = k / p.Cout, co = k % p.Cout;
          int kh = khkw / 5, kw = khkw % 5;
          int y = hi - kh + 2, x = wi - kw + 2;
          if (n < p.CB && y >= 0 && y < p.CH && x >= 0 && x < p.CW)
            v = loadRow8(p.A + (((size_t)n * p.CH + y) * p.CW + x) * p.Cout + co,
                         min(vcnt, p.Cout - co));
        }
      }
    } else if (AMODE == A_T) {
      int kk = c / (BM / 8);
      int i0 = (c % (BM / 8)) * 8;
      int k = kt + kk, m = m0 + i0;
      if (k < kend) v = loadRow8(p.A + (size_t)k * p.lda + m, min(8, p.M - m));
    } else if (AMODE == A_CONV1_FWD) {
      int i = c / (BK / 8);
      int kc = (c % (BK / 8)) * 8;
      int m = m0 + i;
      int n, oy, ox;
      if (m < p.M && kc < 25 && decode_pool_m(p, m, n, oy, ox)) {
#pragma unroll
        for (int e = 0; e < 8; ++e) {
          int k = kt + kc + e;
          if (k < kend && k < 25) {
            int kh = k / 5, kw = k % 5;
            int y = oy + kh - 2, x = ox + kw - 2;
            if (y >= 0 && y < p.CH && x >= 0 && x < p.CW)
              v[e] = p.A[((size_t)n * p.CH + y) * p.CW + x];
          }
        }
      }
    } else {
      int kk = c / (BM / 8);
      int i0 = (c % (BM / 8)) * 8;
      int k = kt + kk, m = m0 + i0;
      if (k < kend && m < p.M) {
        int w_ = k % p.CW, t2 = k / p.CW;
        int h_ = t2 % p.CH, n = t2 / p.CH;
        if (n < p.CB) {
          if (p.Cin % 8 == 0) {
            int khkw = m / p.Cin, ci = m % p.Cin;
            int kh = khkw / 5, kw = khkw % 5;
            int y = h_ + kh - 2, x = w_ + kw - 2;
            if (y >= 0 && y < p.CH && x >= 0 && x < p.CW)
              v = loadRow8(p.A + (((size_t)n * p.CH + y) * p.CW + x) * p.Cin + ci,
                           min(8, p.M - m));
          } else {
#pragma unroll
            for (int e = 0; e < 8; ++e) {
              int me = m + e;
              if (me >= p.M) break;
              int khkw = me / p.Cin, ci = me % p.Cin;
              int kh = khkw / 5, kw = khkw % 5;
              int y = h_ + kh - 2, x = w_ + kw - 2;
              if (y >= 0 && y < p.CH && x >= 0 && x < p.CW)
                v[e] = p.A[(((size_t)n * p.CH + y) * p.CW + x) * p.Cin + ci];
            }
          }
        }
      }
    }
    regs[j] = v;
  }
}

template <int BM, int AMODE, int CH>
DEV void writeA(ushort_t (*As)[LDK], int tid, const short8 (&regs)[CH]) {
#pragma unroll
  for (int j = 0; j < CH; ++j) {
    int c = tid + j * NTHREADS;
    if (AMODE == A_N || AMODE == A_CONV_FWD || AMODE == A_CONV_DX ||
        AMODE == A_CONV1_FWD) {
      int i = c / (BK / 8);
      int kc = (c % (BK / 8)) * 8;
      *reinterpret_cast<short8*>(&As[i][kc]) = regs[j];
    } else {
      int kk = c / (BM / 8);
      int i0 = (c % (BM / 8)) * 8;
#pragma unroll
      for (int e = 0; e < 8; ++e) As[i0 + e][kk] = regs[j][e];
    }
  }
}

template <int BN, int BMODE, int CH>
DEV void loadB(const GemmParams& p, int n0, int kt, int kend, int tid,
               short8 (&regs)[CH]) {
#pragma unroll
  for (int j = 0; j < CH; ++j) {
    int c = tid + j * NTHREADS;
    short8 v = short8{0, 0, 0, 0, 0, 0, 0, 0};
    if (BMODE == B_KMAJ) {
      int kk = c / (BN / 8);
      int j0 = (c % (BN / 8)) * 8;
      int k = kt + kk, n = n0 + j0;
      if (k < kend) v = loadRow8(p.B + (size_t)k * p.ldb + n, min(8, p.N - n));
    } else if (BMODE == B_NMAJ) {
      int i = c / (BK / 8);
      int kc = (c % (BK / 8)) * 8;
      int n = n0 + i, k = kt + kc;
      int vcnt = min(8, kend - k);
      if (n < p.N && vcnt > 0) v = loadRow8(p.B + (size_t)n * p.ldb + k, vcnt);
    } else {
      int i = c / (BK / 8);
      int kc = (c % (BK / 8)) * 8;
      int n = n0 + i, k = kt + kc;
      if (n < p.N && k < kend) {
        int khkw = k / p.Cout, co = k % p.Cout;
        v = loadRow8(p.B + ((size_t)khkw * p.Cin + n) * p.Cout + co,
                     min(min(8, kend - k), p.Cout - co));
      }
    }
    regs[j] = v;
  }
}

template <int BN, int BMODE, int CH>
DEV void writeB(ushort_t (*Bs)[LDK], int tid, const short8 (&regs)[CH]) {
#pragma unroll
  for (int j = 0; j < CH; ++j) {
    int c = tid + j * NTHREADS;
    if (BMODE == B_KMAJ) {
      int kk = c / (BN / 8);
      int j0 = (c % (BN / 8)) * 8;
#pragma unroll
      for (int e = 0; e < 8; ++e) Bs[j0 + e][kk] = regs[j][e];
    } else {
      int i = c / (BK / 8);
      int kc = (c % (BK / 8)) * 8;
      *reinterpret_cast<short8*>(&Bs[i][kc]) = regs[j];
    }
  }
}

template <int BM, int BN, int AMODE, int BMODE, int EPI, int OUT, int PIPE,
          int SWZ = 0>
__global__ __launch_bounds__(NTHREADS)
void gemm_tile_kernel(GemmParams p) {
  constexpr int WM = BM / 2, WN = BN / 2;
  constexpr int MI = WM / 16, NI = WN / 16;
  constexpr int CHA = (BM * BK / 8) / NTHREADS;
  constexpr int CHB = (BN * BK / 8) / NTHREADS;
  constexpr int DB = (PIPE == 1) ? 2 : 1;
  static_assert(CHA >= 1 && CHB >= 1, "tile too small for 256 threads");
  constexpr int A_BYTES = DB * BM * LDK * 2, B_BYTES = DB * BN * LDK * 2;
  __shared__ __align__(16) unsigned char smem[A_BYTES + B_BYTES];
  ushort_t (*As)[BM][LDK] = reinterpret_cast<ushort_t (*)[BM][LDK]>(smem);
  ushort_t (*Bs)[BN][LDK] =
      reinterpret_cast<ushort_t (*)[BN][LDK]>(smem + A_BYTES);
  constexpr bool HAS_DB = (EPI == EPI_UNPOOL || EPI == EPI_MASK_DB);
  __shared__ float dbred[HAS_DB ? BN : 1];
  if (HAS_DB && threadIdx.x < BN) dbred[threadIdx.x] = 0.f;

  const int tid = threadIdx.x;
  constexpr bool UNP = (EPI == EPI_UNPOOL) && (BN % 64 == 0) &&
                       (BM * BN / 16) % NTHREADS == 0 && SWZ == 0;
  constexpr int NAM = UNP ? (BM * BN / 16) / NTHREADS : 1;
  const bool use_lines = UNP && p.unpool_lines;
  uint4 amreg[NAM];
  if (use_lines) {
    const int am_m0 = blockIdx.x * BM, am_n0 = blockIdx.y * BN;
#pragma unroll
    for (int i = 0; i < NAM; ++i) {
      int idx = tid + i * NTHREADS;
      int gr = am_m0 + idx / (BN / 16);
      int gc = am_n0 + (idx % (BN / 16)) * 16;
      amreg[i] = uint4{0x07070707u, 0x07070707u, 0x07070707u, 0x07070707u};
      if (gr < p.M && gc < p.N)
        amreg[i] = *reinterpret_cast<const uint4*>(p.amax + (size_t)gr * p.N + gc);
    }
  }

  const int lane = tid & 63;
  const int wave = tid >> 6;
  const int wr = wave >> 1, wc = wave & 1;
  int bx = blockIdx.x, by = blockIdx.y, bz = blockIdx.z;
  if (SWZ) {
    int gx = (p.M + BM - 1) / BM;
    int gy = (p.N + BN - 1) / BN;
    int total = gx * gy * p.splitk;
    int flat = blockIdx.x;
    int q = total / 8, r = total % 8;
    int xcd = flat % 8, pos = flat / 8;
    int flat2 = (xcd < r ? xcd * (q + 1) : r * (q + 1) + (xcd - r) * q) + pos;
    bx = flat2 % gx;
    int rest = flat2 / gx;
    by = rest % gy;
    bz = rest / gy;
  }
  const int m0 = bx * BM;
  const int n0 = by * BN;

  int ksteps_total = (p.K + BK - 1) / BK;
  int steps_per = (ksteps_total + p.splitk - 1) / p.splitk;
  int kbeg = bz * steps_per * BK;
  int kend = min(p.K, kbeg + steps_per * BK);
  int nt = (kend - kbeg + BK - 1) / BK;
  if (nt <= 0) nt = 0;

  f32x4 acc[MI][NI];
#pragma unroll
  for (int mi = 0; mi < MI; ++mi)
#pragma unroll
    for (int ni = 0; ni < NI; ++ni) acc[mi][ni] = f32x4{0.f, 0.f, 0.f, 0.f};

  const int lrow = lane & 15;
  const int kq = (lane >> 4) * 8;

  short8 ra[CHA], rb[CHB];
  int cur = 0;
  if (PIPE == 2) {
    if (nt > 0) {
      loadA<BM, AMODE, CHA>(p, m0, kbeg, kend, tid, ra);
      loadB<BN, BMODE, CHB>(p, n0, kbeg, kend, tid, rb);
      writeA<BM, AMODE, CHA>(As[0], tid, ra);
      writeB<BN, BMODE, CHB>(Bs[0], tid, rb);
      __syncthreads();
    }
    for (int t = 0; t < nt; ++t) {
      const bool have_next = (t + 1) < nt;
      if (have_next) {
        int kn = kbeg + (t + 1) * BK;
        loadA<BM, AMODE, CHA>(p, m0, kn, kend, tid, ra);
        loadB<BN, BMODE, CHB>(p, n0, kn, kend, tid, rb);
      }
#pragma unroll
      for (int kh = 0; kh < 2; ++kh) {
        short8 af[MI], bf[NI];
#pragma unroll
        for (int mi = 0; mi < MI; ++mi)
          af[mi] = *reinterpret_cast<const short8*>(
              &As[0][wr * WM + mi * 16 + lrow][kh * 32 + kq]);
#pragma unroll
        for (int ni = 0; ni < NI; ++ni)
          bf[ni] = *reinterpret_cast<const short8*>(
              &Bs[0][wc * WN + ni * 16 + lrow][kh * 32 + kq]);
#pragma unroll
        for (int mi = 0; mi < MI; ++mi)
#pragma unroll
          for (int ni = 0; ni < NI; ++ni)
            acc[mi][ni] = __builtin_amdgcn_mfma_f32_16x16x32_bf16(
                af[mi], bf[ni], acc[mi][ni], 0, 0, 0);
      }
      if (have_next) {
        __syncthreads();
        writeA<BM, AMODE, CHA>(As[0], tid, ra);
        writeB<BN, BMODE, CHB>(Bs[0], tid, rb);
        __syncthreads();
      }
    }
    goto epilogue;
  }
  if (PIPE && nt > 0) {
    loadA<BM, AMODE, CHA>(p, m0, kbeg, kend, tid, ra);
    loadB<BN, BMODE, CHB>(p, n0, kbeg, kend, tid, rb);
    writeA<BM, AMODE, CHA>(As[0], tid, ra);
    writeB<BN, BMODE, CHB>(Bs[0], tid, rb);
    __syncthreads();
  }

  for (int t = 0; t < nt; ++t) {
    const bool have_next = PIPE && (t + 1) < nt;
    if (PIPE) {
      if (have_next) {
        int kn = kbeg + (t + 1) * BK;
        loadA<BM, AMODE, CHA>(p, m0, kn, kend, tid, ra);
        loadB<BN, BMODE, CHB>(p, n0, kn, kend, tid, rb);
      }
    } else {
      int kt = kbeg + t * BK;
      loadA<BM, AMODE, CHA>(p, m0, kt, kend, tid, ra);
      loadB<BN, BMODE, CHB>(p, n0, kt, kend, tid, rb);
      writeA<BM, AMODE, CHA>(As[0], tid, ra);
      writeB<BN, BMODE, CHB>(Bs[0], tid, rb);
      __syncthreads();
    }
#pragma unroll
    for (int kh = 0; kh < 2; ++kh) {
      short8 af[MI], bf[NI];
#pragma unroll
      for (int mi = 0; mi < MI; ++mi)
        af[mi] = *reinterpret_cast<const short8*>(
            &As[cur][wr * WM + mi * 16 + lrow][kh * 32 + kq]);
#pragma unroll
      for (int ni = 0; ni < NI; ++ni)
        bf[ni] = *reinterpret_cast<const short8*>(
            &Bs[cur][wc * WN + ni * 16 + lrow][kh * 32 + kq]);
#pragma unroll
      for (int mi = 0; mi < MI; ++mi)
#pragma unroll
        for (int ni = 0; ni < NI; ++ni)
          acc[mi][ni] = __builtin_amdgcn_mfma_f32_16x16x32_bf16(
              af[mi], bf[ni], acc[mi][ni], 0, 0, 0);
    }
    if (PIPE) {
      if (have_next) {
        writeA<BM, AMODE, CHA>(As[cur ^ 1], tid, ra);
        writeB<BN, BMODE, CHB>(Bs[cur ^ 1], tid, rb);
        __syncthreads();
        cur ^= 1;
      }
    } else {
      __syncthreads();
    }
  }

epilogue:
  const int frow = (lane >> 4) * 4;
  const int fcol = lane & 15;
  float dbloc[(EPI == EPI_UNPOOL || EPI == EPI_MASK_DB) ? NI : 1];
  if (EPI == EPI_UNPOOL || EPI == EPI_MASK_DB)
#pragma unroll
    for (int ni = 0; ni < NI; ++ni) dbloc[ni] = 0.f;
  if constexpr (UNP) {
    if (use_lines) {
      constexpr int NJ = BN / 64;
      constexpr int MPP = 2 / NJ;
      constexpr int PR = MPP * 16;
      constexpr int STG = 64 * 4 * 128;
      static_assert(MI % MPP == 0, "passes cover whole mi groups");
      static_assert(STG + BM * BN <= A_BYTES + B_BYTES, "staging fits LDS");
      unsigned char* ams = smem + STG;
      ushort_t* dact = reinterpret_cast<ushort_t*>(p.C);
      const int H2 = p.CHo * 2, W2 = p.CWo * 2;
      const int key = lane >> 4;
      __syncthreads();
#pragma unroll
      for (int i = 0; i < NAM; ++i) {
        int idx = tid + i * NTHREADS;
        int row = idx / (BN / 16), ch = idx % (BN / 16);
        *reinterpret_cast<uint4*>(ams + row * BN +
                                  ((ch ^ ((row >> 2) & 3)) << 4)) = amreg[i];
      }
#pragma unroll
      for (int pass = 0; pass < MI / MPP; ++pass) {
        __syncthreads();
#pragma unroll
        for (int mm = 0; mm < MPP; ++mm) {
          const int mi = pass * MPP + mm;
#pragma unroll
          for (int ni = 0; ni < NI; ++ni) {
            const int colt = wc * WN + ni * 16 + fcol;
            const int j = colt >> 6, c = colt & 63;
#pragma unroll
            for (int r = 0; r < 4; ++r) {
              const int rowt = wr * WM + mi * 16 + frow + r;
              const int lr = wr * PR + mm * 16 + frow + r;
              int pos = ams[rowt * BN + (((colt >> 4) ^ key) << 4) + (colt & 15)];
              float g = pos < 4 ? acc[mi][ni][r] : 0.f;
              dbloc[ni] += g;
              ushort_t gb = f2bf(g);
              unsigned char* sp = smem + ((lr * NJ + j) * 4) * 128 +
                                  (((c >> 3) ^ (key << 1)) << 4) + (c & 7) * 2;
#pragma unroll
              for (int q = 0; q < 4; ++q)
                *reinterpret_cast<ushort_t*>(sp + q * 128) =
                    (pos == q) ? gb : (ushort_t)0;
            }
          }
        }
        __syncthreads();
#pragma unroll
        for (int i = 0; i < 8; ++i) {
          int idx = tid + i * NTHREADS;
          int ch = idx & 7, line = idx >> 3;
          int q = line & 3, slot = line >> 2;
          int j = slot % NJ, lr = slot / NJ;
          int gr = m0 + (lr / PR) * WM + pass * PR + lr % PR;
          int gcol = n0 + j * 64;
          if (gr >= p.M || gcol >= p.N) continue;
          int c0 = gcol % p.Cout, pix = gcol / p.Cout;
          int wo = pix % p.CWo, ho = pix / p.CWo;
          size_t o = (((size_t)gr * H2 + ho * 2 + (q >> 1)) * W2 + wo * 2 +
                      (q & 1)) * p.Cout + c0 + ch * 8;
          *reinterpret_cast<uint4*>(dact + o) = *reinterpret_cast<const uint4*>(
              smem + (slot * 4 + q) * 128 + ((ch ^ (((lr >> 2) & 3) << 1)) << 4));
        }
      }
    }
  }
  if (!use_lines) {
#pragma unroll
  for (int mi = 0; mi < MI; ++mi) {
#pragma unroll
    for (int ni = 0; ni < NI; ++ni) {
      int gc = n0 + wc * WN + ni * 16 + fcol;
      if (gc >= p.N) continue;
      if (EPI == EPI_UNPOOL) {
        int c = gc % p.Cout;
        int pix = gc / p.Cout;
        int wo = pix % p.CWo, ho = pix / p.CWo;
        ushort_t* dact = reinterpret_cast<ushort_t*>(p.C);
        const int H2 = p.CHo * 2, W2 = p.CWo * 2;
#pragma unroll
        for (int r = 0; r < 4; ++r) {
          int gr = m0 + wr * WM + mi * 16 + frow + r;
          if (gr >= p.M) continue;
          size_t qoff = (size_t)gr * p.N + gc;
          int pos = p.amax[qoff];
          float g = pos < 4 ? acc[mi][ni][r] : 0.f;
          dbloc[ni] += g;
          ushort_t gb = f2bf(g);
#pragma unroll
          for (int rr = 0; rr < 2; ++rr)
#pragma unroll
            for (int cc2 = 0; cc2 < 2; ++cc2) {
              size_t o = (((size_t)gr * H2 + ho * 2 + rr) * W2 + wo * 2 +
                          cc2) * p.Cout + c;
              dact[o] = (pos == rr * 2 + cc2) ? gb : (ushort_t)0;
            }
        }
        continue;
      }
      float bias_v = (EPI != EPI_NONE && p.bias) ? p.bias[gc] : 0.f;
      if (EPI == EPI_POOL) {
        int gq = (m0 + wr * WM + mi * 16 + frow) >> 2;
        if (gq * 4 >= p.M) continue;
        float best = -1.0f / 0.0f;
        int barg = 0;
#pragma unroll
        for (int r = 0; r < 4; ++r) {
          float v = acc[mi][ni][r] + bias_v;
          v = v > 0.f ? v : 0.f;
          if (v > best) { best = v; barg = r; }
        }
        ushort_t* Cb = reinterpret_cast<ushort_t*>(p.C);
        Cb[(size_t)gq * p.ldc + gc] = f2bf(best);
        if (p.amax)
          p.amax[(size_t)gq * p.ldc + gc] = (uint8_t)(best > 0.f ? barg : 7);
      } else {
#pragma unroll
        for (int r = 0; r < 4; ++r) {
          int gr = m0 + wr * WM + mi * 16 + frow + r;
          if (gr >= p.M) continue;
          float v = acc[mi][ni][r];
          if (EPI == EPI_MASK_DB) {
            float a = bf2f(p.actm[(size_t)gr * p.ldc + gc]);
            v = (a > 0.f) ? v * p.p_keep : 0.f;
            dbloc[ni] += v;
          }
          if (EPI != EPI_NONE && EPI != EPI_MASK_DB) v += bias_v;
          if (EPI == EPI_BIAS_RELU || EPI == EPI_BIAS_RELU_DROP)
            v = v > 0.f ? v : 0.f;
          if (EPI == EPI_BIAS_RELU_DROP) {
            uint64_t off = p.offset_dev ? (uint64_t)*p.offset_dev : p.offset;
            float u = philox_uniform(p.seed, off, (uint64_t)gr * p.N + gc);
            v = (u < p.p_keep) ? v / p.p_keep : 0.f;
          }
          if (OUT == OUT_BF16) {
            reinterpret_cast<ushort_t*>(p.C)[(size_t)gr * p.ldc + gc] = f2bf(v);
          } else if (OUT == OUT_F32_SLICES || OUT == OUT_F32_SLICES_FIX) {
            float* outp = reinterpret_cast<float*>(p.C) +
                          (size_t)bz * p.M * p.ldc;
            if (OUT == OUT_F32_SLICES_FIX)
              __hip_atomic_store(&outp[(size_t)gr * p.ldc + gc], v,
                                 __ATOMIC_RELAXED, __HIP_MEMORY_SCOPE_AGENT);
            else
              outp[(size_t)gr * p.ldc + gc] = v;
          } else {
            atomicAdd(reinterpret_cast<float*>(p.C) + (size_t)gr * p.ldc + gc, v);
          }
        }
      }
    }
  }
  }
  if constexpr (OUT == OUT_F32_SLICES_FIX) {
    static_assert(BM == 64 && BN == 64, "fix-up thread map is 64 x 64");
    {
      __shared__ unsigned last_flag;
      __syncthreads();
      unsigned* tk = p.tickets + (size_t)by * gridDim.x + bx;
      if (tid == 0) {
        __builtin_amdgcn_fence(__ATOMIC_RELEASE, "agent");
        last_flag = (atomicAdd(tk, 1u) == (unsigned)p.splitk - 1u) ? 1u : 0u;
      }
      __syncthreads();
      if (last_flag) {
        __builtin_amdgcn_fence(__ATOMIC_ACQUIRE, "agent");
        const size_t plane = (size_t)p.M * p.ldc;
        const float* acc0 = reinterpret_cast<const float*>(p.C);
        const uint64_t off = p.offset_dev ? (uint64_t)*p.offset_dev : p.offset;
        const int gr = m0 + (tid >> 2);
        const int gcb = n0 + (tid & 3) * 16;
        const bool ok[2] = {gr < p.M && gcb < p.N, gr < p.M && gcb + 8 < p.N};
        float sum[2][8];
#pragma unroll
        for (int h = 0; h < 2; ++h)
#pragma unroll
          for (int e = 0; e < 8; ++e) sum[h][e] = 0.f;
        for (int s0 = 0; s0 < p.splitk; s0 += 4) {
          union { unsigned long long q; float f[2]; } t[4][2][4];
#pragma unroll
          for (int ds = 0; ds < 4; ++ds)
#pragma unroll
            for (int h = 0; h < 2; ++h)
#pragma unroll
              for (int e2 = 0; e2 < 4; ++e2) {
                t[ds][h][e2].q = 0ull;
                if (ok[h] && s0 + ds < p.splitk)
                  t[ds][h][e2].q = __hip_atomic_load(
                      reinterpret_cast<const unsigned long long*>(
                          acc0 + (size_t)(s0 + ds) * plane +
                          (size_t)gr * p.N + gcb + h * 8 + e2 * 2),
                      __ATOMIC_RELAXED, __HIP_MEMORY_SCOPE_AGENT);
              }
#pragma unroll
          for (int ds = 0; ds < 4; ++ds)
            if (s0 + ds < p.splitk)
#pragma unroll
              for (int h = 0; h < 2; ++h)
#pragma unroll
                for (int e = 0; e < 8; ++e)
                  sum[h][e] += t[ds][h][e >> 1].f[e & 1];
        }
#pragma unroll
        for (int h = 0; h < 2; ++h) {
          const int gc = gcb + h * 8;
          if (!ok[h]) continue;
          union { ushort_t u[8]; uint4 v; } o;
#pragma unroll
          for (int e = 0; e < 8; ++e) {
            const size_t i = (size_t)gr * p.N + gc + e;
            float v = sum[h][e];
            v += p.bias[gc + e];
            if (p.relu) v = v > 0.f ? v : 0.f;
            if (p.p_keep < 1.0f) {
              float u = philox_uniform(p.seed, off, (uint64_t)i);
              v = (u < p.p_keep) ? v / p.p_keep : 0.f;
            }
            o.u[e] = f2bf(v);
          }
          *reinterpret_cast<uint4*>(p.Y + (size_t)gr * p.N + gc) = o.v;
        }
        if (tid == 0)
          __hip_atomic_store(tk, 0u, __ATOMIC_RELAXED, __HIP_MEMORY_SCOPE_AGENT);
      }
    }
  }
  if (EPI == EPI_UNPOOL || EPI == EPI_MASK_DB) {
#pragma unroll
    for (int ni = 0; ni < NI; ++ni) {
      int colb = wc * WN + ni * 16 + fcol;
      if (dbloc[ni] != 0.f) atomicAdd(&dbred[colb], dbloc[ni]);
    }
    __syncthreads();
    if (p.db && (int)threadIdx.x < BN) {
      int gc = n0 + (int)threadIdx.x;
      float v = dbred[threadIdx.x];
      int idx = (EPI == EPI_UNPOOL) ? gc % p.Cout : gc;
      if (gc < p.N && v != 0.f) atomicAdd(&p.db[idx], v);
    }
  }
}

#include <hip/hip_runtime_api.h>

static inline int cdiv_host(int a, int b) { return (a + b - 1) / b; }

#define GEMM_ENTRY(name, BM, BN, AM, BMo, EPI, OUT, PIPE)                   \
  void name(const GemmParams& p, hipStream_t s) {                            \
    dim3 grid(cdiv_host(p.M, BM), cdiv_host(p.N, BN), p.splitk);             \
    hipLaunchKernelGGL((gemm_tile_kernel<BM, BN, AM, BMo, EPI, OUT, PIPE>),  \
                       grid, dim3(NTHREADS), 0, s, p);                       \
  }
#define GEMM_ENTRY_SWZ(name, BM, BN, AM, BMo, EPI, OUT, PIPE)                \
  void name(const GemmParams& p, hipStream_t s) {                            \
    dim3 grid(cdiv_host(p.M, BM) * cdiv_host(p.N, BN) * p.splitk);           \
    hipLaunchKernelGGL((gemm_tile_kernel<BM, BN, AM, BMo, EPI, OUT, PIPE,    \
                                         1>),                                \
                       grid, dim3(NTHREADS), 0, s, p);                       \
  }

GEMM_ENTRY(gemm_fwd_bias_128, 128, 128, A_N, B_KMAJ, EPI_BIAS, OUT_BF16, 1)
GEMM_ENTRY(gemm_fwd_bias_64, 64, 64, A_N, B_KMAJ, EPI_BIAS, OUT_BF16, 1)
GEMM_ENTRY(gemm_fwd_relu_128, 128, 128, A_N, B_KMAJ, EPI_BIAS_RELU, OUT_BF16, 1)
GEMM_ENTRY(gemm_fwd_relu_64, 64, 64, A_N, B_KMAJ, EPI_BIAS_RELU, OUT_BF16, 1)
GEMM_ENTRY(gemm_fwd_drop_128, 128, 128, A_N, B_KMAJ, EPI_BIAS_RELU_DROP, OUT_BF16, 1)
GEMM_ENTRY(gemm_fwd_drop_64, 64, 64, A_N, B_KMAJ, EPI_BIAS_RELU_DROP, OUT_BF16, 1)
GEMM_ENTRY(gemm_dx_128, 128, 128, A_N, B_NMAJ, EPI_NONE, OUT_BF16, 1)
GEMM_ENTRY(gemm_dx_64, 64, 64, A_N, B_NMAJ, EPI_NONE, OUT_BF16, 1)
GEMM_ENTRY(gemm_dx_unpool_128, 128, 128, A_N, B_NMAJ, EPI_UNPOOL, OUT_BF16, 1)
GEMM_ENTRY(gemm_dx_unpool_64, 64, 64, A_N, B_NMAJ, EPI_UNPOOL, OUT_BF16, 1)
GEMM_ENTRY(gemm_dx_mask_128, 128, 128, A_N, B_NMAJ, EPI_MASK_DB, OUT_BF16, 1)
GEMM_ENTRY(gemm_dx_mask_64, 64, 64, A_N, B_NMAJ, EPI_MASK_DB, OUT_BF16, 1)
GEMM_ENTRY_SWZ(gemm_dw_128, 128, 128, A_T, B_KMAJ, EPI_NONE, OUT_F32_ATOMIC, 2)
GEMM_ENTRY_SWZ(gemm_dw_64, 64, 64, A_T, B_KMAJ, EPI_NONE, OUT_F32_ATOMIC, 2)
GEMM_ENTRY(gemm_fwd_bias_128_bt, 128, 128, A_N, B_NMAJ, EPI_BIAS, OUT_BF16, 1)
GEMM_ENTRY(gemm_fwd_bias_64_bt, 64, 64, A_N, B_NMAJ, EPI_BIAS, OUT_BF16, 1)
GEMM_ENTRY(gemm_fwd_relu_128_bt, 128, 128, A_N, B_NMAJ, EPI_BIAS_RELU, OUT_BF16, 1)
GEMM_ENTRY(gemm_fwd_relu_64_bt, 64, 64, A_N, B_NMAJ, EPI_BIAS_RELU, OUT_BF16, 1)
GEMM_ENTRY(gemm_fwd_drop_128_bt, 128, 128, A_N, B_NMAJ, EPI_BIAS_RELU_DROP, OUT_BF16, 1)
GEMM_ENTRY(gemm_fwd_drop_64_bt, 64, 64, A_N, B_NMAJ, EPI_BIAS_RELU_DROP, OUT_BF16, 1)
GEMM_ENTRY(gemm_fwd_slices_64, 64, 64, A_N, B_KMAJ, EPI_NONE, OUT_F32_SLICES, 1)
GEMM_ENTRY(gemm_fwd_slices_64_bt, 64, 64, A_N, B_NMAJ, EPI_NONE, OUT_F32_SLICES, 1)
GEMM_ENTRY(gemm_fwd_slices_fix_64, 64, 64, A_N, B_KMAJ, EPI_NONE, OUT_F32_SLICES_FIX, 1)
GEMM_ENTRY(gemm_fwd_slices_fix_64_bt, 64, 64, A_N, B_NMAJ, EPI_NONE, OUT_F32_SLICES_FIX, 1)
GEMM_ENTRY(conv_fwd_pool, 128, 64, A_CONV_FWD, B_KMAJ, EPI_POOL, OUT_BF16, 0)
GEMM_ENTRY(conv_fwd_pool_bt, 128, 64, A_CONV_FWD, B_NMAJ, EPI_POOL, OUT_BF16, 0)
GEMM_ENTRY(conv1_fwd_pool, 128, 64, A_CONV1_FWD, B_KMAJ, EPI_POOL, OUT_BF16, 0)
GEMM_ENTRY(conv_dx_gemm, 128, 32, A_CONV_DX, B_CONV_DX_W, EPI_NONE, OUT_BF16, 0)
GEMM_ENTRY_SWZ(conv_dw_gemm, 128, 64, A_CONV_DW, B_KMAJ, EPI_NONE, OUT_F32_ATOMIC, 2)
GEMM_ENTRY_SWZ(conv1_dw_gemm, 32, 32, A_CONV_DW, B_KMAJ, EPI_NONE, OUT_F32_ATOMIC, 2)
```

csrc/kernels.h:

```cpp
#pragma once
#include <hip/hip_runtime.h>
#include <stdint.h>

struct GemmParams {
  const unsigned short* A;
  const unsigned short* B;
  const float* bias;
  void* C;
  uint8_t* amax;
  int M, N, K;
  int lda, ldb, ldc;
  int splitk;
  int CB, CH, CW, CHo, CWo, Cin, Cout;
  float p_keep;
  uint64_t seed, offset;
  const long* offset_dev;
  float* db;
  const unsigned short* actm;
  int unpool_lines;
  unsigned* tickets;
  unsigned short* Y;
  int relu;
};

void gemm_fwd_bias_128(const GemmParams&, hipStream_t);
void gemm_fwd_bias_64(const GemmParams&, hipStream_t);
void gemm_fwd_relu_128(const GemmParams&, hipStream_t);
void gemm_fwd_relu_64(const GemmParams&, hipStream_t);
void gemm_fwd_drop_128(const GemmParams&, hipStream_t);
void gemm_fwd_drop_64(const GemmParams&, hipStream_t);
void gemm_dx_128(const GemmParams&, hipStream_t);
void gemm_dx_64(const GemmParams&, hipStream_t);
void gemm_dx_unpool_128(const GemmParams&, hipStream_t);
void gemm_dx_unpool_64(const GemmParams&, hipStream_t);
void gemm_dx_mask_128(const GemmParams&, hipStream_t);
void gemm_dx_mask_64(const GemmParams&, hipStream_t);
void gemm_dw_128(const GemmParams&, hipStream_t);
void gemm_dw_64(const GemmParams&, hipStream_t);
void conv_fwd_pool(const GemmParams&, hipStream_t);
void conv1_fwd_pool(const GemmParams&, hipStream_t);
void conv_dx_gemm(const GemmParams&, hipStream_t);
void conv_dw_gemm(const GemmParams&, hipStream_t);
void conv_dw_tr(const GemmParams&, hipStream_t);
void gemm_dw_tr(const GemmParams&, int tbm, int bn, bool single_writer,
                hipStream_t);

void launch_relu_drop_bwd(const unsigned short* dy, const unsigned short* y,
                          unsigned short* dyeff, float* db, int B, int N,
                          float inv_keep, int apply_mask, hipStream_t);
void launch_pool_bwd_scatter(const unsigned short* dy, const unsigned short* y,
                             const uint8_t* amax, unsigned short* dact,
                             float* db, int Mpool, int C, int H, int W, int Wo,
                             hipStream_t);
#define SOFTMAX_MAX_BLOCKS 4096
void launch_softmax_xent(const unsigned short* logits, const long* labels,
                         unsigned short* dlogits, float* out, int B, int C,
                         float* db, float inv_n, float* part,
                         unsigned* ticket, hipStream_t);
void launch_sgd_step(float* master, float* grad, unsigned short* shadow,
                     int has_shadow, long n, float lr_scale, float dc_keep,
                     uint64_t seed, uint64_t offset, float* momentum, float mu,
                     hipStream_t);
void launch_sgd_step_dev(float* master, float* grad,
                         unsigned short* shadow, int has_shadow, long n,
                         const float* lr_scale_dev, float dc_keep,
                         uint64_t seed, const long* offset_dev,
                         float* momentum, float mu, int zero_grad,
                         hipStream_t);
void launch_conv1_dw_pooled(const unsigned short* x, const unsigned short* dyp,
                            const uint8_t* am, float* dw, float* db, int NB,
                            int H, int W, int Cout, hipStream_t s);
void launch_grad_mask(float* g, long n, long base, float keep, uint64_t seed,
                      uint64_t step, uint64_t rank, const long* step_dev,
                      hipStream_t s);
void launch_step_advance(long* step_dev, float* lr_scale_dev, float lr0,
                         float decay, int decay_steps, float inv_contrib,
                         hipStream_t);
void launch_batch_gather(const uint8_t* img, const uint8_t* lab,
                         const unsigned short* lut, unsigned short* x,
                         long* y, uint32_t N, uint32_t B, uint64_t seed,
                         uint64_t step, const long* step_dev, hipStream_t);
void launch_batch_gather_aug(const uint8_t* img, const uint8_t* lab,
                             const unsigned short* lut, const int* table,
                             uint32_t T, unsigned short* x, long* y,
                             uint32_t N, uint32_t B, uint64_t seed,
                             uint64_t step, const long* step_dev,
                             hipStream_t);
void launch_range_gather(const uint8_t* img, const uint8_t* lab,
                         const unsigned short* lut, unsigned short* x,
                         long* y, uint32_t N, uint32_t B, uint64_t start,
                         const long* start_dev, hipStream_t);
void launch_softmax_eval(const unsigned short* logits, const long* labels,
                         float* loss_sum, int* counts, uint8_t* pred,
                         long* cursor_dev, int B, int C, float* part,
                         unsigned* ticket, hipStream_t);
void launch_transpose_bf16(const unsigned short* src, unsigned short* dst,
                           int R, int C, hipStream_t);
struct TransposeDesc {
  const unsigned short* src;
  unsigned short* dst;
  int R, C;
};
struct TransposeBatchArgs {
  TransposeDesc d[4];
  int tile0[4];
  int n, total;
  int do_advance;
  long* step_dev;
  float* lr_scale_dev;
  float lr0, decay, inv_contrib;
  int decay_steps;
};
void launch_transpose_bf16_batch(const TransposeDesc* descs, int n,
                                 hipStream_t);
void launch_transpose_bf16_batch_adv(const TransposeDesc* descs, int n,
                                     long* step_dev, float* lr_scale_dev,
                                     float lr0, float decay, int decay_steps,
                                     float inv_contrib, hipStream_t);
void launch_conv1_direct_fwd(const unsigned short* x, const unsigned short* w,
                             const float* bias, unsigned short* y,
                             uint8_t* amax, int NB, int H, int W, int Cout,
                             hipStream_t);
void gemm_fwd_bias_128_bt(const GemmParams&, hipStream_t);
void gemm_fwd_bias_64_bt(const GemmParams&, hipStream_t);
void gemm_fwd_relu_128_bt(const GemmParams&, hipStream_t);
void gemm_fwd_relu_64_bt(const GemmParams&, hipStream_t);
void gemm_fwd_drop_128_bt(const GemmParams&, hipStream_t);
void gemm_fwd_drop_64_bt(const GemmParams&, hipStream_t);
void conv_fwd_pool_bt(const GemmParams&, hipStream_t);
void conv1_dw_gemm(const GemmParams&, hipStream_t);
bool conv_slab_supported(int H, int W, int Cin, int Cout);
void launch_conv_fwd_slab(const unsigned short* x, const unsigned short* w,
                          const float* bias, unsigned short* y, uint8_t* amax,
                          int NB, int H, int W, int Cin, int Cout, hipStream_t);
void launch_conv_dx_slab(const unsigned short* dact, const unsigned short* w,
                         unsigned short* dx, int NB, int H, int W, int Cin,
                         int Cout, hipStream_t);
void launch_conv_dw_slab(const unsigned short* x, const unsigned short* dact,
                         float* dw, int NB, int H, int W, int Cin, int Cout,
                         hipStream_t);
bool conv1_slab_supported(int H, int W, int Cin, int Cout);
void launch_conv1_dw_slab(const unsigned short* x, const unsigned short* dact,
                          float* dw, int NB, int H, int W, int Cout,
                          hipStream_t);
void launch_conv1_dw_direct(const unsigned short* x,
                            const unsigned short* dact, float* dw, int NB,
                            int H, int W, int Cout, hipStream_t s);
bool conv1_mfma_supported(int H, int W, int Cin, int Cout);
bool conv1_mfma_enabled();
int conv1_mfma_dw_group(int NB);
void launch_conv1_mfma_fwd(const unsigned short* x, const unsigned short* w,
                           const float* bias, unsigned short* y,
                           uint8_t* amax, int NB, hipStream_t);
void launch_conv1_mfma_dw(const unsigned short* x, const unsigned short* dyp,
                          const uint8_t* am, float* dw, float* db, int NB,
                          hipStream_t);
bool conv2_dw_slab_supported(int H, int W, int Cin, int Cout);
bool conv2_dw_slab_enabled();
int conv2_dw_group(int NB);
void launch_conv2_dw_slab(const unsigned short* x, const unsigned short* dact,
                          float* dw, int NB, hipStream_t);
void gemm_fwd_slices_64(const GemmParams&, hipStream_t);
void gemm_fwd_slices_64_bt(const GemmParams&, hipStream_t);
void gemm_fwd_slices_fix_64(const GemmParams&, hipStream_t);
void gemm_fwd_slices_fix_64_bt(const GemmParams&, hipStream_t);
void launch_fwd_epilogue(const float* acc, const float* bias,
                         unsigned short* y, int M, int N, int slices,
                         int relu, float p_keep, uint64_t seed,
                         uint64_t offset, const long* offset_dev,
                         hipStream_t);
```

distributedmnist_amd/engine/fused_step.py:

```python

from __future__ import annotations

import torch
import torch.distributed as dist

from .. import _C


class FusedLeNetStep:
    def __init__(self, trainer):
        t = trainer
        m = t.model
        from ..models import LeNet5
        assert isinstance(m, LeNet5), "fused step is LeNet-specific"
        assert t.compute_dtype == torch.bfloat16 and t.device.type == "cuda"
        assert m.shadows and m.shadows_T, "fused step needs bf16 shadows"
        self.t = t
        self.ext = _C.ext()
        import os as _os
        if _os.environ.get("DMNIST_OVERLAP"):
            self.overlap_level = int(_os.environ["DMNIST_OVERLAP"])
        elif _os.environ.get("DMNIST_TWO_STREAM"):
            self.overlap_level = 2
        elif _os.environ.get("DMNIST_SINGLE_STREAM"):
            self.overlap_level = 0
        else:
            self.overlap_level = 0 if t.flags.batch_size < 4096 else 2
        self.single_stream = self.overlap_level == 0
        self.side = None if self.single_stream else torch.cuda.Stream()
        self.p_keep = 0.5
        self.seed = t.flags.seed
        fp = t.fp
        fc0 = fp.offsets[fp.names.index("fc1_w")]
        self.fc_offset = fc0
        self.conv_slice = fp.flat_grad[:fc0]
        self.fc_slice = fp.flat_grad[fc0:]
        self.overlap_allreduce = t.world > 1 and dist.is_initialized()

    def _fork(self, a, b):
        if not self.single_stream:
            a.wait_stream(b)

    def __call__(self, x, labels, step_dev):
        ext = self.ext
        m = self.t.model
        sh, shT = m.shadows, m.shadows_T
        B = x.shape[0]

        def gv(name):
            return getattr(m, name).grad

        s0 = torch.cuda.current_stream()
        s1 = s0 if self.single_stream else self.side

        y1, am1 = ext.conv_pool_fwd(x, sh["conv1_w"], m.conv1_b, None)
        y2, am2 = ext.conv_pool_fwd(y1, sh["conv2_w"], m.conv2_b,
                                    shT["conv2_w"])
        h2 = y2.view(B, 7 * 7 * 64)
        a1 = ext.linear_act_fwd_dev(h2, sh["fc1_w"], m.fc1_b, True,
                                    self.p_keep, self.seed, step_dev,
                                    shT["fc1_w"])
        logits = ext.linear_act_fwd(a1, sh["fc2_w"], m.fc2_b, False, 1.0,
                                    0, 0, shT["fc2_w"])
        loss, acc, dl = ext.softmax_xent_fwd(logits, labels,
                                             db_out=gv("fc2_b"),
                                             inv_n=1.0 / B)

        self._fork(s1, s0)
        with torch.cuda.stream(s1):
            ext.linear_dw_into(a1, dl, gv("fc2_w"))
        dyeff1 = ext.linear_dx_mask(dl, sh["fc2_w"], a1, gv("fc1_b"),
                                    self.p_keep)
        self._fork(s1, s0)
        with torch.cuda.stream(s1):
            ext.linear_dw_into(h2, dyeff1, gv("fc1_w"))
            if self.overlap_allreduce:
                self.t.engine.wire_allreduce(self.fc_slice,
                                             start=self.fc_offset)
        dact2 = ext.linear_dx_unpool(dyeff1, sh["fc1_w"], am2,
                                     gv("conv2_b"), 7, 7, 64)
        sW = s1 if self.overlap_level >= 2 else s0
        if sW is not s0:
            self._fork(sW, s0)
        with torch.cuda.stream(sW):
            ext.conv_dw_into(y1, dact2, gv("conv2_w"))
        dxc = ext.conv_dx(dact2, sh["conv2_w"], 32)

        ext.conv1_dw_pooled(x, dxc, am1, gv("conv1_w"), gv("conv1_b"))

        self._fork(s0, s1)
        if self.overlap_allreduce:
            self.t.engine.wire_allreduce(self.conv_slice, start=0)
        self._keep = (a1, h2, dyeff1, dl, y1, dact2)
        return loss, acc

    def stage_fc(self, x, labels, step_dev):
        ext = self.ext
        m = self.t.model
        sh, shT = m.shadows, m.shadows_T
        B = x.shape[0]

        def gv(name):
            return getattr(m, name).grad

        s0 = torch.cuda.current_stream()
        s1 = s0 if self.single_stream else self.side
        y1, am1 = ext.conv_pool_fwd(x, sh["conv1_w"], m.conv1_b, None)
        y2, am2 = ext.conv_pool_fwd(y1, sh["conv2_w"], m.conv2_b,
                                    shT["conv2_w"])
        h2 = y2.view(B, 7 * 7 * 64)
        a1 = ext.linear_act_fwd_dev(h2, sh["fc1_w"], m.fc1_b, True,
                                    self.p_keep, self.seed, step_dev,
                                    shT["fc1_w"])
        logits = ext.linear_act_fwd(a1, sh["fc2_w"], m.fc2_b, False, 1.0,
                                    0, 0, shT["fc2_w"])
        loss, acc, dl = ext.softmax_xent_fwd(logits, labels,
                                             db_out=gv("fc2_b"),
                                             inv_n=1.0 / B)
        self._fork(s1, s0)
        with torch.cuda.stream(s1):
            ext.linear_dw_into(a1, dl, gv("fc2_w"))
        dyeff1 = ext.linear_dx_mask(dl, sh["fc2_w"], a1, gv("fc1_b"),
                                    self.p_keep)
        self._fork(s1, s0)
        with torch.cuda.stream(s1):
            ext.linear_dw_into(h2, dyeff1, gv("fc1_w"))
        dact2 = ext.linear_dx_unpool(dyeff1, sh["fc1_w"], am2,
                                     gv("conv2_b"), 7, 7, 64)
        s0.wait_stream(s1)
        self._stash = (x, y1, am1, dact2)
        self._keep = (a1, h2, dyeff1, dl)
        return loss, acc

    def stage_conv(self):
        ext = self.ext
        m = self.t.model

        def gv(name):
            return getattr(m, name).grad

        x, y1, am1, dact2 = self._stash
        s0 = torch.cuda.current_stream()
        s1 = s0 if self.single_stream else self.side
        sW = s1 if self.overlap_level >= 2 else s0
        if sW is not s0:
            self._fork(sW, s0)
        with torch.cuda.stream(sW):
            ext.conv_dw_into(y1, dact2, gv("conv2_w"))
        dxc = ext.conv_dx(dact2, m.shadows["conv2_w"], 32)
        ext.conv1_dw_pooled(x, dxc, am1, gv("conv1_w"), gv("conv1_b"))
        self._fork(s0, s1)
        self._keep2 = (dact2,)
```

Before: 3.810 million images/sec.

## Keep conv2 gradient pooled and unpool inside conv2 dX/dW kernels

Instead of having the fc1 dX GEMM scatter into a full-resolution 14x14x64 unpooled gradient, the GEMM now writes only the 7x7x64 pooled gradient, masked by the argmax byte, plus the conv2 bias gradient. The conv2 dX slab kernel and the conv2 dW slab kernel each read the pooled gradient and argmax bytes and expand the 2x2 windows into LDS themselves. This cuts global writes and reads of the mostly-zero unpooled tensor, at the cost of extra selection work and an extra argmax read in two consumer kernels. It is on by default and can be disabled through an environment variable.

```diff
diff --git a/csrc/bindings.cpp b/csrc/bindings.cpp
--- a/csrc/bindings.cpp
+++ b/csrc/bindings.cpp
@@ -474,6 +474,39 @@
   return dact;
 }
 
+#define POOLED_DX_BIG_TILES 150
+
+torch::Tensor linear_dx_pooled(torch::Tensor dyeff, torch::Tensor w,
+                               torch::Tensor amax, torch::Tensor db_out,
+                               int64_t Ho, int64_t Wo, int64_t C,
+                               int64_t tile) {
+  CHECK_BF16(dyeff); CHECK_CONTIG(dyeff); CHECK_BF16(w); CHECK_CONTIG(w);
+  CHECK_CONTIG(amax);
+  TORCH_CHECK(amax.scalar_type() == at::kByte, "amax must be uint8");
+  int B = dyeff.size(0), N = dyeff.size(1), K = w.size(0);
+  TORCH_CHECK(K == Ho * Wo * C, "linear_dx_pooled: K != Ho*Wo*C");
+  TORCH_CHECK(w.size(1) == N, "linear_dx_pooled: w is [K][N]");
+  TORCH_CHECK(amax.numel() == (int64_t)B * K, "linear_dx_pooled: amax shape");
+  TORCH_CHECK(tile == 0 || tile == 64 || tile == 128,
+              "linear_dx_pooled: tile is 0, 64 or 128");
+  auto gp = torch::empty({B, (int)Ho, (int)Wo, (int)C}, dyeff.options());
+  GemmParams p{};
+  p.A = bf16_ptr(dyeff); p.B = bf16_ptr(w);
+  p.C = gp.data_ptr();
+  p.M = B; p.N = K; p.K = N;
+  p.lda = N; p.ldb = N; p.ldc = K;
+  p.splitk = 1;
+  p.CHo = Ho; p.CWo = Wo; p.Cout = C;
+  p.amax = amax.data_ptr<uint8_t>();
+  p.db = db_out.defined() ? db_out.data_ptr<float>() : nullptr;
+  p.unpool_lines = K % 16 == 0 && ((uintptr_t)p.amax & 15) == 0 &&
+                   ((uintptr_t)p.C & 15) == 0;
+  bool big = cdiv(B, 128) * cdiv(K, 128) >= POOLED_DX_BIG_TILES;
+  if (tile) big = tile == 128;
+  (big ? gemm_dx_poolmask_128 : gemm_dx_poolmask_64)(p, cur_stream());
+  return gp;
+}
+
 torch::Tensor linear_dx_mask(torch::Tensor dyeff, torch::Tensor w,
                              torch::Tensor actm, torch::Tensor db_out,
                              double p_keep) {
@@ -604,6 +637,51 @@
   return dx;
 }
 
+static void check_pooled(const torch::Tensor& gp, const torch::Tensor& am) {
+  CHECK_CUDA(gp); CHECK_BF16(gp); CHECK_CONTIG(gp);
+  CHECK_CUDA(am); CHECK_CONTIG(am);
+  TORCH_CHECK(am.scalar_type() == at::kByte, "am must be uint8");
+  TORCH_CHECK(gp.dim() == 4 && gp.size(1) == 7 && gp.size(2) == 7 &&
+                  gp.size(3) == 64,
+              "pooled conv2 backward: gp is [NB][7][7][64]");
+  TORCH_CHECK(am.numel() == gp.numel(), "am / gp shape mismatch");
+  TORCH_CHECK(((uintptr_t)gp.data_ptr() & 15) == 0 &&
+                  ((uintptr_t)am.data_ptr() & 7) == 0,
+              "pooled conv2 backward: gp 16 B / am 8 B alignment");
+}
+
+torch::Tensor conv_dx_pooled(torch::Tensor gp, torch::Tensor am,
+                             torch::Tensor w, int64_t Cin, int64_t force_db) {
+  check_pooled(gp, am);
+  CHECK_BF16(w); CHECK_CONTIG(w);
+  TORCH_CHECK(Cin == 32 && w.numel() == 25 * 32 * 64,
+              "conv_dx_pooled: LeNet conv2 shapes only");
+  TORCH_CHECK(force_db >= 0 && force_db <= 2, "force_db is 0, 1 or 2");
+  int NB = gp.size(0);
+  auto dx = torch::empty({NB, 14, 14, 32}, gp.options());
+  if (NB > 0)
+    launch_conv_dx_slab_pooled(bf16_ptr(gp), am.data_ptr<uint8_t>(),
+                               bf16_ptr(w), bf16_mut(dx), NB, (int)force_db,
+                               cur_stream());
+  return dx;
+}
+
+void conv_dw_pooled_into(torch::Tensor x, torch::Tensor gp, torch::Tensor am,
+                         torch::Tensor dw_out) {
+  check_pooled(gp, am);
+  CHECK_CUDA(x); CHECK_BF16(x); CHECK_CONTIG(x);
+  CHECK_F32(dw_out); CHECK_CONTIG(dw_out);
+  TORCH_CHECK(x.dim() == 4 && x.size(0) == gp.size(0) && x.size(1) == 14 &&
+                  x.size(2) == 14 && x.size(3) == 32,
+              "conv_dw_pooled_into: x is [NB][14][14][32]");
+  TORCH_CHECK(dw_out.numel() == 25 * 32 * 64, "conv_dw_pooled_into: dw size");
+  TORCH_CHECK(((uintptr_t)x.data_ptr() & 15) == 0, "x 16 B alignment");
+  launch_conv2_dw_slab_pooled(bf16_ptr(x), bf16_ptr(gp),
+                              am.data_ptr<uint8_t>(),
+                              dw_out.data_ptr<float>(), (int)x.size(0),
+                              cur_stream());
+}
+
 std::vector<torch::Tensor> softmax_xent_fwd(torch::Tensor logits,
                                             torch::Tensor labels,
                                             c10::optional<torch::Tensor> db_out,
@@ -955,6 +1033,22 @@
         "dx GEMM fused with maxpool2x2 backward scatter + conv db",
         py::arg("dyeff"), py::arg("w"), py::arg("amax"),
         py::arg("db_out"), py::arg("Ho"), py::arg("Wo"), py::arg("C"));
+  m.def("linear_dx_pooled", &linear_dx_pooled,
+        "dx GEMM masked by the pool argmax byte + conv db: pooled gradient",
+        py::arg("dyeff"), py::arg("w"), py::arg("amax"),
+        py::arg("db_out"), py::arg("Ho"), py::arg("Wo"), py::arg("C"),
+        py::arg("tile") = 0);
+  m.def("linear_dx_pooled_tile", [](int64_t B, int64_t K) {
+          return (int64_t)(cdiv((int)B, 128) * cdiv((int)K, 128) >=
+                                   POOLED_DX_BIG_TILES ? 128 : 64);
+        }, "tile linear_dx_pooled picks for dyeff[B,*], w[K,*]");
+  m.def("conv_dx_pooled", &conv_dx_pooled,
+        "conv2 dX from the pooled gradient + pool argmax bytes",
+        py::arg("gp"), py::arg("am"), py::arg("w"), py::arg("Cin"),
+        py::arg("force_db") = 0);
+  m.def("conv_dw_pooled_into", &conv_dw_pooled_into,
+        "conv2 dW from the pooled gradient + pool argmax bytes, into bucket",
+        py::arg("x"), py::arg("gp"), py::arg("am"), py::arg("dw_out"));
   m.def("linear_dw_plan", [](int64_t K, int64_t N, int64_t B) {
     DwPlan pl = linear_dw_plan((int)K, (int)N, (int)B);
     return std::make_tuple(pl.tbm, pl.bn, pl.splitk);
diff --git a/csrc/common.h b/csrc/common.h
--- a/csrc/common.h
+++ b/csrc/common.h
@@ -81,6 +81,16 @@
   return r.s;
 }
 
+DEV short8 pool_bwd_select(short8 g, uint2 a, int pos) {
+  short8 v;
+#pragma unroll
+  for (int e = 0; e < 8; ++e) {
+    unsigned b = ((e < 4 ? a.x : a.y) >> (8 * (e & 3))) & 0xffu;
+    v[e] = b == (unsigned)pos ? g[e] : (short)0;
+  }
+  return v;
+}
+
 typedef short bf16x2_t __attribute__((__vector_size__(2 * sizeof(short))));
 DEV float dot2bf(unsigned a, unsigned b, float c) {
   union U { unsigned u; bf16x2_t v; };
diff --git a/csrc/conv2_dw_slab.hip b/csrc/conv2_dw_slab.hip
--- a/csrc/conv2_dw_slab.hip
+++ b/csrc/conv2_dw_slab.hip
@@ -7,6 +7,7 @@
 #define C2_MG 8
 #define C2_XIMG (14 * 14 * 32)
 #define C2_DIMG (14 * 14 * 64)
+#define C2_PIMG (7 * 7 * 64)
 
 static __device__ __align__(16) unsigned short c2_zero_page[8];
 
@@ -15,14 +16,16 @@
 
 extern __shared__ __align__(16) ushort_t c2_lds[];
 
-template <int KHB, int NBUF>
+template <int KHB, int NBUF, bool POOLED = false>
 __global__ __launch_bounds__(256, (KHB == 1 && NBUF == 1) ? 3 : 1)
 void conv2_dw_slab_kernel(const ushort_t* __restrict__ x,
                           const ushort_t* __restrict__ dact,
-                          float* __restrict__ dw, int NB, int G) {
+                          float* __restrict__ dw, int NB, int G,
+                          const uint8_t* __restrict__ am) {
+  static_assert(!POOLED || (KHB == 1 && NBUF == 1), "pooled: shipped form only");
   constexpr int NRX = 13 + KHB;
   constexpr int XPIX = C2_MG + NRX * 16 + C2_MG;
-  constexpr int NJOB = NRX + 28;
+  constexpr int NJOB = POOLED ? NRX : NRX + 28;
   constexpr int NQ = (NJOB + 3) / 4;
   constexpr int NKB = 5 / KHB;
   constexpr int KS_UNROLL = KHB == 1 ? 7 : 1;
@@ -44,6 +47,12 @@
     int t = tid & 63;
     int o = (t < 32) ? t * 8 : (C2_MG + NRX * 16) * 32 + (t - 32) * 8;
     *reinterpret_cast<short8*>(X + (tid >> 6) * BUF + o) =
+        short8{0, 0, 0, 0, 0, 0, 0, 0};
+  }
+
+  if (POOLED && tid < 224) {
+    int k = (tid >> 4) * 16 + 14 + ((tid >> 3) & 1);
+    *reinterpret_cast<short8*>(D + k * 64 + (tid & 7) * 8) =
         short8{0, 0, 0, 0, 0, 0, 0, 0};
   }
 
@@ -116,6 +125,35 @@
     if (NBUF == 1) {
       __syncthreads();
       issue(0, img0 + g);
+      if (POOLED) {
+        const ushort_t* gi = dact + (size_t)(img0 + g) * C2_PIMG;
+        const uint8_t* ai = am + (size_t)(img0 + g) * C2_PIMG;
+        short8 gv[2];
+        uint2 av[2];
+#pragma unroll
+        for (int j = 0; j < 2; ++j) {
+          int c = tid + j * 256;
+          if (c < 49 * 8) {
+            gv[j] = *reinterpret_cast<const short8*>(gi + c * 8);
+            av[j] = *reinterpret_cast<const uint2*>(ai + c * 8);
+          }
+        }
+#pragma unroll
+        for (int j = 0; j < 2; ++j) {
+          int c = tid + j * 256;
+          if (c < 49 * 8) {
+            int chunk = c & 7, win = c >> 3;
+            int wy = win / 7, wx = win - wy * 7;
+#pragma unroll
+            for (int pos = 0; pos < 4; ++pos) {
+              int k = (2 * wy + (pos >> 1)) * 16 + 2 * wx + (pos & 1);
+              *reinterpret_cast<short8*>(D + k * 64 +
+                                         ((chunk ^ c2_dswz(k)) << 3)) =
+                  pool_bwd_select(gv[j], av[j], pos);
+            }
+          }
+        }
+      }
     }
     asm volatile("s_waitcnt vmcnt(0)" ::: "memory");
     __syncthreads();
@@ -184,19 +222,21 @@
   return G < 1 ? 1 : G;
 }
 
-template <int KHB, int NBUF>
+template <int KHB, int NBUF, bool POOLED = false>
 static void c2_launch(const unsigned short* x, const unsigned short* dact,
-                      float* dw, int NB, int G, int blocks, hipStream_t s) {
+                      float* dw, int NB, int G, int blocks, hipStream_t s,
+                      const uint8_t* am = nullptr) {
   constexpr int BYTES = NBUF * ((C2_MG * 2 + (13 + KHB) * 16) * 32 + 224 * 64) * 2;
   if (BYTES > 65536) {
     static const hipError_t granted = hipFuncSetAttribute(
-        reinterpret_cast<const void*>(&conv2_dw_slab_kernel<KHB, NBUF>),
+        reinterpret_cast<const void*>(
+            &conv2_dw_slab_kernel<KHB, NBUF, POOLED>),
         hipFuncAttributeMaxDynamicSharedMemorySize, BYTES);
     if (granted != hipSuccess)
       throw std::runtime_error("conv2_dw_slab: LDS size not granted");
   }
-  hipLaunchKernelGGL((conv2_dw_slab_kernel<KHB, NBUF>), dim3(blocks),
-                     dim3(256), BYTES, s, x, dact, dw, NB, G);
+  hipLaunchKernelGGL((conv2_dw_slab_kernel<KHB, NBUF, POOLED>), dim3(blocks),
+                     dim3(256), BYTES, s, x, dact, dw, NB, G, am);
 }
 
 void launch_conv2_dw_slab(const unsigned short* x, const unsigned short* dact,
@@ -218,3 +258,13 @@
   else
     c2_launch<1, 1>(x, dact, dw, NB, G, g8 * 5, s);
 }
+
+void launch_conv2_dw_slab_pooled(const unsigned short* x,
+                                 const unsigned short* gp, const uint8_t* am,
+                                 float* dw, int NB, hipStream_t s) {
+  if (NB <= 0) return;
+  int G = conv2_dw_group(NB);
+  int groups = (NB + G - 1) / G;
+  int g8 = (groups + 7) / 8 * 8;
+  c2_launch<1, 1, true>(x, gp, dw, NB, G, g8 * 5, s, am);
+}
diff --git a/csrc/conv_slab.hip b/csrc/conv_slab.hip
--- a/csrc/conv_slab.hip
+++ b/csrc/conv_slab.hip
@@ -179,11 +179,13 @@
   }
 }
 
-template <int H, int W, int CIN, int COUT, int DB = 2, int PAD = 8>
+template <int H, int W, int CIN, int COUT, int DB = 2, int PAD = 8,
+          bool POOLED = false>
 __global__ __launch_bounds__(NTHREADS)
 void conv_dx_slab_kernel(const u16* __restrict__ dact,
                          const u16* __restrict__ w,
-                         u16* __restrict__ dx, int NB) {
+                         u16* __restrict__ dx, int NB,
+                         const uint8_t* __restrict__ am) {
   constexpr int HP = H + 4, WP = W + 4;
   constexpr int M = H * W;
   constexpr int BM = 224;
@@ -216,6 +218,47 @@
     glds16(src, &Bs[buf][wave * 8][0]);
   };
 
+  if (POOLED) {
+    constexpr int HO = H / 2, WO = W / 2;
+    const u16* gi = dact + (size_t)img * HO * WO * COUT;
+    const uint8_t* ai = am + (size_t)img * HO * WO * COUT;
+    constexpr int NWJ = HO * WO * (COUT / 8);
+    constexpr int NJ = (NWJ + NTHREADS - 1) / NTHREADS;
+    short8 g[NJ];
+    uint2 a[NJ];
+#pragma unroll
+    for (int j = 0; j < NJ; ++j) {
+      int c = tid + j * NTHREADS;
+      if (c < NWJ) {
+        g[j] = *reinterpret_cast<const short8*>(gi + (size_t)c * 8);
+        a[j] = *reinterpret_cast<const uint2*>(ai + (size_t)c * 8);
+      }
+    }
+    for (int c = tid; c < HP * WP * (COUT / 8); c += NTHREADS) {
+      int co = (c % (COUT / 8)) * 8;
+      int pix = c / (COUT / 8);
+      int xx = pix % WP, yy = pix / WP;
+      int sy = yy - 2, sx = xx - 2;
+      if (!(sy >= 0 && sy < H && sx >= 0 && sx < W))
+        *reinterpret_cast<short8*>(&slab[(yy * WP + xx) * PST + co]) =
+            short8{0, 0, 0, 0, 0, 0, 0, 0};
+    }
+#pragma unroll
+    for (int j = 0; j < NJ; ++j) {
+      int c = tid + j * NTHREADS;
+      if (c < NWJ) {
+        int co = (c % (COUT / 8)) * 8;
+        int win = c / (COUT / 8);
+        int wx = win % WO, wy = win / WO;
+#pragma unroll
+        for (int pos = 0; pos < 4; ++pos) {
+          int yy = 2 * wy + (pos >> 1) + 2, xx = 2 * wx + (pos & 1) + 2;
+          *reinterpret_cast<short8*>(&slab[(yy * WP + xx) * PST + co]) =
+              pool_bwd_select(g[j], a[j], pos);
+        }
+      }
+    }
+  } else {
   for (int c = tid; c < HP * WP * (COUT / 8); c += NTHREADS) {
     int co = (c % (COUT / 8)) * 8;
     int pix = c / (COUT / 8);
@@ -225,6 +268,7 @@
     if (sy >= 0 && sy < H && sx >= 0 && sx < W)
       v = *reinterpret_cast<const short8*>(di + ((size_t)sy * W + sx) * COUT + co);
     *reinterpret_cast<short8*>(&slab[(yy * WP + xx) * PST + co]) = v;
+  }
   }
 
   int arow_off[MI];
@@ -478,20 +522,36 @@
   if (H == 14 && W == 14 && Cin == 32 && Cout == 64) {
     if (getenv("DMNIST_DX_PAIR"))
       hipLaunchKernelGGL((conv_dx_slab_kernel<14, 14, 32, 64, 3>), dim3(NB),
-                         dim3(NTHREADS), 0, s, dact, w, dx, NB);
+                         dim3(NTHREADS), 0, s, dact, w, dx, NB,
+                         (const uint8_t*)nullptr);
     else if (NB < 2048)
       hipLaunchKernelGGL((conv_dx_slab_kernel<14, 14, 32, 64, 2>), dim3(NB),
-                         dim3(NTHREADS), 0, s, dact, w, dx, NB);
+                         dim3(NTHREADS), 0, s, dact, w, dx, NB,
+                         (const uint8_t*)nullptr);
     else if (getenv("DMNIST_DX_HIOCC"))
       hipLaunchKernelGGL((conv_dx_slab_hi_occ_kernel<14, 14, 32, 64>),
                          dim3(NB), dim3(NTHREADS), 0, s, dact, w, dx, NB);
     else if (getenv("DMNIST_DX_DB2SLIM"))
       hipLaunchKernelGGL((conv_dx_slab_kernel<14, 14, 32, 64, 2, 4>),
-                         dim3(NB), dim3(NTHREADS), 0, s, dact, w, dx, NB);
+                         dim3(NB), dim3(NTHREADS), 0, s, dact, w, dx, NB,
+                         (const uint8_t*)nullptr);
     else
       hipLaunchKernelGGL((conv_dx_slab_kernel<14, 14, 32, 64, 1>), dim3(NB),
-                         dim3(NTHREADS), 0, s, dact, w, dx, NB);
-  }
+                         dim3(NTHREADS), 0, s, dact, w, dx, NB,
+                         (const uint8_t*)nullptr);
+  }
+}
+
+void launch_conv_dx_slab_pooled(const unsigned short* gp, const uint8_t* am,
+                                const unsigned short* w, unsigned short* dx,
+                                int NB, int force_db, hipStream_t s) {
+  int db = force_db ? force_db : (NB < 2048 ? 2 : 1);
+  if (db == 2)
+    hipLaunchKernelGGL((conv_dx_slab_kernel<14, 14, 32, 64, 2, 8, true>),
+                       dim3(NB), dim3(NTHREADS), 0, s, gp, w, dx, NB, am);
+  else
+    hipLaunchKernelGGL((conv_dx_slab_kernel<14, 14, 32, 64, 1, 8, true>),
+                       dim3(NB), dim3(NTHREADS), 0, s, gp, w, dx, NB, am);
 }
 
 template <int H, int W, int CIN, int COUT, int G, int ABL = 0>
diff --git a/csrc/gemm_tile.hip b/csrc/gemm_tile.hip
--- a/csrc/gemm_tile.hip
+++ b/csrc/gemm_tile.hip
@@ -16,7 +16,7 @@
   B_CONV_DX_W = 2,
 };
 enum Epi { EPI_NONE = 0, EPI_BIAS = 1, EPI_BIAS_RELU = 2, EPI_BIAS_RELU_DROP = 3,
-           EPI_POOL = 4, EPI_UNPOOL = 5, EPI_MASK_DB = 6 };
+           EPI_POOL = 4, EPI_UNPOOL = 5, EPI_MASK_DB = 6, EPI_POOLMASK_DB = 7 };
 enum OutKind { OUT_BF16 = 0, OUT_F32_ATOMIC = 1, OUT_F32_SLICES = 2,
                OUT_F32_SLICES_FIX = 3 };
 
@@ -223,15 +223,18 @@
   ushort_t (*As)[BM][LDK] = reinterpret_cast<ushort_t (*)[BM][LDK]>(smem);
   ushort_t (*Bs)[BN][LDK] =
       reinterpret_cast<ushort_t (*)[BN][LDK]>(smem + A_BYTES);
-  constexpr bool HAS_DB = (EPI == EPI_UNPOOL || EPI == EPI_MASK_DB);
+  constexpr bool HAS_DB = (EPI == EPI_UNPOOL || EPI == EPI_MASK_DB ||
+                           EPI == EPI_POOLMASK_DB);
   __shared__ float dbred[HAS_DB ? BN : 1];
   if (HAS_DB && threadIdx.x < BN) dbred[threadIdx.x] = 0.f;
 
   const int tid = threadIdx.x;
   constexpr bool UNP = (EPI == EPI_UNPOOL) && (BN % 64 == 0) &&
                        (BM * BN / 16) % NTHREADS == 0 && SWZ == 0;
-  constexpr int NAM = UNP ? (BM * BN / 16) / NTHREADS : 1;
-  const bool use_lines = UNP && p.unpool_lines;
+  constexpr bool PML = (EPI == EPI_POOLMASK_DB) &&
+                       (BM * BN / 16) % NTHREADS == 0 && SWZ == 0;
+  constexpr int NAM = (UNP || PML) ? (BM * BN / 16) / NTHREADS : 1;
+  const bool use_lines = (UNP || PML) && p.unpool_lines;
   uint4 amreg[NAM];
   if (use_lines) {
     const int am_m0 = blockIdx.x * BM, am_n0 = blockIdx.y * BN;
@@ -383,8 +386,8 @@
 epilogue:
   const int frow = (lane >> 4) * 4;
   const int fcol = lane & 15;
-  float dbloc[(EPI == EPI_UNPOOL || EPI == EPI_MASK_DB) ? NI : 1];
-  if (EPI == EPI_UNPOOL || EPI == EPI_MASK_DB)
+  float dbloc[HAS_DB ? NI : 1];
+  if (HAS_DB)
 #pragma unroll
     for (int ni = 0; ni < NI; ++ni) dbloc[ni] = 0.f;
   if constexpr (UNP) {
@@ -454,6 +457,47 @@
       }
     }
   }
+  if constexpr (PML) {
+    if (use_lines) {
+      constexpr int SST = (BN + 8) * 2, AST = BN + 16;
+      constexpr int STG = BM * SST;
+      static_assert(STG + BM * AST <= A_BYTES + B_BYTES, "staging fits LDS");
+      unsigned char* ams = smem + STG;
+      __syncthreads();
+#pragma unroll
+      for (int i = 0; i < NAM; ++i) {
+        int idx = tid + i * NTHREADS;
+        int row = idx / (BN / 16), ch = idx % (BN / 16);
+        *reinterpret_cast<uint4*>(ams + row * AST + ch * 16) = amreg[i];
+      }
+      __syncthreads();
+#pragma unroll
+      for (int mi = 0; mi < MI; ++mi)
+#pragma unroll
+        for (int ni = 0; ni < NI; ++ni) {
+          const int colt = wc * WN + ni * 16 + fcol;
+#pragma unroll
+          for (int r = 0; r < 4; ++r) {
+            const int rowt = wr * WM + mi * 16 + frow + r;
+            int pos = ams[rowt * AST + colt];
+            float g = pos < 4 ? acc[mi][ni][r] : 0.f;
+            dbloc[ni] += g;
+            *reinterpret_cast<ushort_t*>(smem + rowt * SST + colt * 2) = f2bf(g);
+          }
+        }
+      __syncthreads();
+      ushort_t* gp = reinterpret_cast<ushort_t*>(p.C);
+#pragma unroll
+      for (int i = 0; i < (BM * BN / 8) / NTHREADS; ++i) {
+        int idx = tid + i * NTHREADS;
+        int row = idx / (BN / 8), ch = idx % (BN / 8);
+        int gr = m0 + row, gc = n0 + ch * 8;
+        if (gr >= p.M || gc >= p.N) continue;
+        *reinterpret_cast<uint4*>(gp + (size_t)gr * p.ldc + gc) =
+            *reinterpret_cast<const uint4*>(smem + row * SST + ch * 16);
+      }
+    }
+  }
   if (!use_lines) {
 #pragma unroll
   for (int mi = 0; mi < MI; ++mi) {
@@ -509,12 +553,18 @@
           int gr = m0 + wr * WM + mi * 16 + frow + r;
           if (gr >= p.M) continue;
           float v = acc[mi][ni][r];
+          if (EPI == EPI_POOLMASK_DB) {
+            int pos = p.amax[(size_t)gr * p.N + gc];
+            v = pos < 4 ? v : 0.f;
+            dbloc[ni] += v;
+          }
           if (EPI == EPI_MASK_DB) {
             float a = bf2f(p.actm[(size_t)gr * p.ldc + gc]);
             v = (a > 0.f) ? v * p.p_keep : 0.f;
             dbloc[ni] += v;
           }
-          if (EPI != EPI_NONE && EPI != EPI_MASK_DB) v += bias_v;
+          if (EPI != EPI_NONE && EPI != EPI_MASK_DB && EPI != EPI_POOLMASK_DB)
+            v += bias_v;
           if (EPI == EPI_BIAS_RELU || EPI == EPI_BIAS_RELU_DROP)
             v = v > 0.f ? v : 0.f;
           if (EPI == EPI_BIAS_RELU_DROP) {
@@ -613,7 +663,7 @@
       }
     }
   }
-  if (EPI == EPI_UNPOOL || EPI == EPI_MASK_DB) {
+  if (HAS_DB) {
 #pragma unroll
     for (int ni = 0; ni < NI; ++ni) {
       int colb = wc * WN + ni * 16 + fcol;
@@ -623,7 +673,8 @@
     if (p.db && (int)threadIdx.x < BN) {
       int gc = n0 + (int)threadIdx.x;
       float v = dbred[threadIdx.x];
-      int idx = (EPI == EPI_UNPOOL) ? gc % p.Cout : gc;
+      int idx = (EPI == EPI_UNPOOL || EPI == EPI_POOLMASK_DB) ? gc % p.Cout
+                                                               : gc;
       if (gc < p.N && v != 0.f) atomicAdd(&p.db[idx], v);
     }
   }
@@ -657,6 +708,8 @@
 GEMM_ENTRY(gemm_dx_64, 64, 64, A_N, B_NMAJ, EPI_NONE, OUT_BF16, 1)
 GEMM_ENTRY(gemm_dx_unpool_128, 128, 128, A_N, B_NMAJ, EPI_UNPOOL, OUT_BF16, 1)
 GEMM_ENTRY(gemm_dx_unpool_64, 64, 64, A_N, B_NMAJ, EPI_UNPOOL, OUT_BF16, 1)
+GEMM_ENTRY(gemm_dx_poolmask_128, 128, 128, A_N, B_NMAJ, EPI_POOLMASK_DB, OUT_BF16, 1)
+GEMM_ENTRY(gemm_dx_poolmask_64, 64, 64, A_N, B_NMAJ, EPI_POOLMASK_DB, OUT_BF16, 1)
 GEMM_ENTRY(gemm_dx_mask_128, 128, 128, A_N, B_NMAJ, EPI_MASK_DB, OUT_BF16, 1)
 GEMM_ENTRY(gemm_dx_mask_64, 64, 64, A_N, B_NMAJ, EPI_MASK_DB, OUT_BF16, 1)
 GEMM_ENTRY_SWZ(gemm_dw_128, 128, 128, A_T, B_KMAJ, EPI_NONE, OUT_F32_ATOMIC, 2)
diff --git a/csrc/kernels.h b/csrc/kernels.h
--- a/csrc/kernels.h
+++ b/csrc/kernels.h
@@ -33,6 +33,8 @@
 void gemm_dx_64(const GemmParams&, hipStream_t);
 void gemm_dx_unpool_128(const GemmParams&, hipStream_t);
 void gemm_dx_unpool_64(const GemmParams&, hipStream_t);
+void gemm_dx_poolmask_128(const GemmParams&, hipStream_t);
+void gemm_dx_poolmask_64(const GemmParams&, hipStream_t);
 void gemm_dx_mask_128(const GemmParams&, hipStream_t);
 void gemm_dx_mask_64(const GemmParams&, hipStream_t);
 void gemm_dw_128(const GemmParams&, hipStream_t);
@@ -136,6 +138,9 @@
 void launch_conv_dx_slab(const unsigned short* dact, const unsigned short* w,
                          unsigned short* dx, int NB, int H, int W, int Cin,
                          int Cout, hipStream_t);
+void launch_conv_dx_slab_pooled(const unsigned short* gp, const uint8_t* am,
+                                const unsigned short* w, unsigned short* dx,
+                                int NB, int force_db, hipStream_t);
 void launch_conv_dw_slab(const unsigned short* x, const unsigned short* dact,
                          float* dw, int NB, int H, int W, int Cin, int Cout,
                          hipStream_t);
@@ -160,6 +165,9 @@
 int conv2_dw_group(int NB);
 void launch_conv2_dw_slab(const unsigned short* x, const unsigned short* dact,
                           float* dw, int NB, hipStream_t);
+void launch_conv2_dw_slab_pooled(const unsigned short* x,
+                                 const unsigned short* gp, const uint8_t* am,
+                                 float* dw, int NB, hipStream_t);
 void gemm_fwd_slices_64(const GemmParams&, hipStream_t);
 void gemm_fwd_slices_64_bt(const GemmParams&, hipStream_t);
 void gemm_fwd_slices_fix_64(const GemmParams&, hipStream_t);
diff --git a/distributedmnist_amd/engine/fused_step.py b/distributedmnist_amd/engine/fused_step.py
--- a/distributedmnist_amd/engine/fused_step.py
+++ b/distributedmnist_amd/engine/fused_step.py
@@ -27,6 +27,7 @@
         else:
             self.overlap_level = 0 if t.flags.batch_size < 4096 else 2
         self.single_stream = self.overlap_level == 0
+        self.pool2_fused = _os.environ.get("DMNIST_POOL2_FUSED", "1") != "0"
         self.side = None if self.single_stream else torch.cuda.Stream()
         self.p_keep = 0.5
         self.seed = t.flags.seed
@@ -77,22 +78,40 @@
             if self.overlap_allreduce:
                 self.t.engine.wire_allreduce(self.fc_slice,
                                              start=self.fc_offset)
-        dact2 = ext.linear_dx_unpool(dyeff1, sh["fc1_w"], am2,
-                                     gv("conv2_b"), 7, 7, 64)
+        g2 = self._fc1_dx(dyeff1, am2)
         sW = s1 if self.overlap_level >= 2 else s0
         if sW is not s0:
             self._fork(sW, s0)
         with torch.cuda.stream(sW):
-            ext.conv_dw_into(y1, dact2, gv("conv2_w"))
-        dxc = ext.conv_dx(dact2, sh["conv2_w"], 32)
+            self._conv2_dw(y1, g2, am2)
+        dxc = self._conv2_dx(g2, am2)
 
         ext.conv1_dw_pooled(x, dxc, am1, gv("conv1_w"), gv("conv1_b"))
 
         self._fork(s0, s1)
         if self.overlap_allreduce:
             self.t.engine.wire_allreduce(self.conv_slice, start=0)
-        self._keep = (a1, h2, dyeff1, dl, y1, dact2)
+        self._keep = (a1, h2, dyeff1, dl, y1, g2, am2)
         return loss, acc
+
+    def _fc1_dx(self, dyeff1, am2):
+        m = self.t.model
+        f = (self.ext.linear_dx_pooled if self.pool2_fused
+             else self.ext.linear_dx_unpool)
+        return f(dyeff1, m.shadows["fc1_w"], am2, m.conv2_b.grad, 7, 7, 64)
+
+    def _conv2_dw(self, y1, g2, am2):
+        dw = self.t.model.conv2_w.grad
+        if self.pool2_fused:
+            self.ext.conv_dw_pooled_into(y1, g2, am2, dw)
+        else:
+            self.ext.conv_dw_into(y1, g2, dw)
+
+    def _conv2_dx(self, g2, am2):
+        w = self.t.model.shadows["conv2_w"]
+        if self.pool2_fused:
+            return self.ext.conv_dx_pooled(g2, am2, w, 32)
+        return self.ext.conv_dx(g2, w, 32)
 
     def stage_fc(self, x, labels, step_dev):
         ext = self.ext
@@ -125,10 +144,9 @@
         self._fork(s1, s0)
         with torch.cuda.stream(s1):
             ext.linear_dw_into(h2, dyeff1, gv("fc1_w"))
-        dact2 = ext.linear_dx_unpool(dyeff1, sh["fc1_w"], am2,
-                                     gv("conv2_b"), 7, 7, 64)
+        g2 = self._fc1_dx(dyeff1, am2)
         s0.wait_stream(s1)
-        self._stash = (x, y1, am1, dact2)
+        self._stash = (x, y1, am1, g2, am2)
         self._keep = (a1, h2, dyeff1, dl)
         return loss, acc
 
@@ -139,15 +157,15 @@
         def gv(name):
             return getattr(m, name).grad
 
-        x, y1, am1, dact2 = self._stash
+        x, y1, am1, g2, am2 = self._stash
         s0 = torch.cuda.current_stream()
         s1 = s0 if self.single_stream else self.side
         sW = s1 if self.overlap_level >= 2 else s0
         if sW is not s0:
             self._fork(sW, s0)
         with torch.cuda.stream(sW):
-            ext.conv_dw_into(y1, dact2, gv("conv2_w"))
-        dxc = ext.conv_dx(dact2, m.shadows["conv2_w"], 32)
+            self._conv2_dw(y1, g2, am2)
+        dxc = self._conv2_dx(g2, am2)
         ext.conv1_dw_pooled(x, dxc, am1, gv("conv1_w"), gv("conv1_b"))
         self._fork(s0, s1)
-        self._keep2 = (dact2,)
+        self._keep2 = (g2, am2)
```

Result: faster. 3.875 million images/sec, median of 6 (+1.7%).
